# mutiann/few-shot-transformer-tts

Hardware: AMD Instinct MI355X
Metric: padded mel-frames/sec, full training step (fwd+loss+bwd+allreduce+Adam) (higher is better)
Workload: dtype bf16; 1 GPU; LJSpeech-shaped (BASELINE configs[1]) packed batch per GPU: B=14 S=114 T=582, default hparams (83.5M params), dropout on, single speaker/language; global_batch=14, seq_len=582, parallelism=dp1

## Files before the change

few-shot-transformer-tts_amd/b2s_hip/lib.py:

```python
import ctypes as C
import os

os.environ.setdefault("GPU_MAX_HW_QUEUES", "8")

import torch

_HERE = os.path.dirname(os.path.abspath(__file__))
LIB_PATH = os.environ.get("B2S_LIB_PATH") or os.path.join(os.path.dirname(_HERE), "libb2s_hip.so")

_lib = None


class B2SError(RuntimeError):
    pass


class Config(C.Structure):
    _fields_ = [(n, C.c_int32) for n in (
        "num_mels", "vocab_size", "embed_size", "encoder_hidden", "decoder_hidden",
        "n_encoder_layer", "n_decoder_layer", "n_attention_head",
        "prenet_hidden", "postnet_hidden", "n_postnet_layer",
        "multi_speaker", "max_num_speaker", "speaker_embedding_size",
        "multi_lingual", "max_num_language", "language_embedding_size")] + [
        ("transformer_dropout_rate", C.c_float), ("decoder_dropout_rate", C.c_float),
        ("reg_weight", C.c_float), ("compute_dtype", C.c_int32),
        ("guided_attention_weight", C.c_float), ("guided_attention_sigma", C.c_float), ("freeze_encoder", C.c_int32)]


class GemmDesc(C.Structure):
    _fields_ = [(n, C.c_int32) for n in ("dtype", "trans_a", "trans_b", "M", "N", "K", "lda", "ldb", "ldc", "c_fp32",
                                         "batch", "batch_inner")] + \
               [(n, C.c_int64) for n in ("a_bs_o", "a_bs_i", "b_bs_o", "b_bs_i", "c_bs_o", "c_bs_i")] + \
               [("alpha", C.c_float), ("relu", C.c_int32), ("accumulate", C.c_int32), ("drop_p", C.c_float),
                ("seed", C.c_uint64), ("conv_cin_a", C.c_int32), ("conv_T", C.c_int32), ("conv_dw_cin", C.c_int32),
                ("rows_per_batch", C.c_int32)]


P = C.c_void_p
_PROTOS = {
    "b2s_last_error": (C.c_char_p, []),
    "b2s_version": (C.c_int, []),
    "b2s_model_create": (C.c_int, [C.POINTER(Config), C.POINTER(P)]),
    "b2s_model_destroy": (None, [P]),
    "b2s_model_num_tensors": (C.c_int, [P]),
    "b2s_model_tensor_info": (C.c_int, [P, C.c_int, C.c_char_p, C.c_int, C.POINTER(C.c_int64), C.POINTER(C.c_int), C.POINTER(C.c_int)]),
    "b2s_model_bind": (C.c_int, [P, C.POINTER(P), C.POINTER(P), C.c_int]),
    "b2s_model_sync_weights": (C.c_int, [P, P, C.c_int]),
    "b2s_encoder_ws_bytes": (C.c_size_t, [P, C.c_int, C.c_int]),
    "b2s_encoder_forward": (C.c_int, [P, P, P, P, P, C.c_int, C.c_int, C.c_int, C.c_uint64, P, C.c_size_t, P, P, C.POINTER(P)]),
    "b2s_encoder_backward": (C.c_int, [P, P, P, P]),
    "b2s_decoder_ws_bytes": (C.c_size_t, [P, C.c_int, C.c_int, C.c_int]),
    "b2s_decoder_forward": (C.c_int, [P, P, P, P, P, C.c_int, C.c_int, C.c_int, C.c_int, C.c_uint64, P, C.c_size_t, P, P, P, P, C.POINTER(P)]),
    "b2s_decoder_backward": (C.c_int, [P, P, P, P, P, C.c_int, P, P, P]),
    "b2s_decoder_guided_loss": (C.c_int, [P, P, P, P, P]),
    "b2s_decoder_alignment": (C.c_int, [P, P, C.c_int, C.c_int, P, P]),
    "b2s_postnet_ws_bytes": (C.c_size_t, [P, C.c_int, C.c_int]),
    "b2s_postnet_forward": (C.c_int, [P, P, P, P, C.c_int, C.c_int, C.c_int, C.c_uint64, P, C.c_size_t, P, P, C.POINTER(P)]),
    "b2s_postnet_backward": (C.c_int, [P, P, P, P, C.c_int, P]),
    "b2s_ctx_free": (None, [P]),
    "b2s_loss_forward": (C.c_int, [P, P, P, P, P, P, C.c_int, C.c_int, P, P, P, P]),
    "b2s_loss_backward": (C.c_int, [P, P, P, P, P, P, C.c_int, C.c_int, P, P, P, P, P]),
    "b2s_l2_backward": (C.c_int, [P, P, P]),
    "b2s_adam_bind": (C.c_int, [P, C.POINTER(P), C.POINTER(P), C.c_int]),
    "b2s_adam_step": (C.c_int, [P, C.c_float, C.c_int, C.c_float, C.c_float, C.c_float, C.c_float, C.c_float, P]),
    "b2s_zero_grads": (C.c_int, [P, P, C.c_int]),
    "b2s_model_set_grad_slot_padding": (C.c_int, [P, C.c_int]),
    "b2s_gemm": (C.c_int, [C.POINTER(GemmDesc), P, P, P, P, P, P, P, P]),
    "b2s_gemm_splitk": (C.c_int, [C.POINTER(GemmDesc), C.c_int, P, P, P, P, C.c_size_t, P]),
    "b2s_layernorm_forward": (C.c_int, [C.c_int, P, P, P, P, P, P, C.c_int, C.c_int, C.c_float, P]),
    "b2s_layernorm_backward": (C.c_int, [C.c_int, P, P, P, P, P, P, P, P, C.c_int, C.c_int, P]),
    "b2s_attention_ws_bytes": (C.c_size_t, [C.c_int, C.c_int, C.c_int, C.c_int, C.c_int]),
    "b2s_attention_forward": (C.c_int, [C.c_int, P, C.c_int, P, C.c_int, P, C.c_int, P, C.c_int, C.c_int, C.c_int, C.c_int,
                                        C.c_int, C.c_int, C.c_int, P, P, C.c_int64, C.c_int64, C.c_float, C.c_uint64, P, P, P, P]),
    "b2s_attention_backward": (C.c_int, [C.c_int, P, C.c_int, P, C.c_int, P, C.c_int, P, C.c_int, P, P, P, C.c_int, P, C.c_int,
                                         P, C.c_int, C.c_int, C.c_int, C.c_int, C.c_int, C.c_int, C.c_float, C.c_uint64, P, P]),
    "b2s_flash_attention_forward": (C.c_int, [C.c_int, P, C.c_int, P, C.c_int, P, C.c_int, P, C.c_int, C.c_int, C.c_int, C.c_int, C.c_int,
                                              C.c_int, C.c_int, P, C.c_float, C.c_uint64, P, P]),
    "b2s_flash_attention_backward": (C.c_int, [C.c_int, P, P, C.c_int, P, C.c_int, P, C.c_int, P, C.c_int, P, P, P, C.c_int, P, C.c_int,
                                               P, C.c_int, C.c_int, C.c_int, C.c_int, C.c_int, C.c_int, C.c_int, P, C.c_float,
                                               C.c_uint64, P]),
    "b2s_flash_attention_align": (C.c_int, [C.c_int, P, C.c_int, P, C.c_int, P, C.c_int, C.c_int, C.c_int, C.c_int, C.c_int, C.c_int, P, P,
                                            P]),
    "b2s_align_from_probs": (C.c_int, [C.c_int, P, P, C.c_int, C.c_int, C.c_int, C.c_int, P]),
    "b2s_add3": (C.c_int, [P, P, P, P, C.c_int64, P]),
    "b2s_cast": (C.c_int, [C.c_int, P, P, C.c_int64, P]),
    "b2s_cast_back": (C.c_int, [C.c_int, P, P, C.c_int64, P]),
    "b2s_decode_ws_bytes": (C.c_size_t, [P, C.c_int, C.c_int, C.c_int, C.c_int]),
    "b2s_decode_begin": (C.c_int, [P, P, P, C.c_int, C.c_int, C.c_int, C.c_int, C.c_uint64, C.c_int, P, C.c_size_t, P, C.POINTER(P)]),
    "b2s_decode_run": (C.c_int, [P, P, C.c_int, C.c_int, P]),
    "b2s_decode_status": (C.c_int, [P, C.POINTER(C.c_int), C.POINTER(C.c_int), P]),
    "b2s_decode_fetch": (C.c_int, [P, P, C.c_int, P, P, P]),
    "b2s_decode_alignment": (C.c_int, [P, P, C.c_int, C.c_int, C.c_int, P, P]),
    "b2s_decode_end": (None, [P]),
    "b2s_model_second_stream": (C.c_void_p, [P]),
    "b2s_model_set_side_stream": (C.c_int, [P, P]),
    "b2s_gemm_set_tile_policy": (C.c_int, [C.c_int]),
    "b2s_model_backward_abort": (C.c_int, [P, P]),
    "b2s_model_mark_grads_ready": (C.c_int, [P]),
    "b2s_adam_shard": (C.c_int, [P, P, C.POINTER(C.c_int64), C.POINTER(C.c_int64), C.c_int]),
    "b2s_param_wire": (C.c_int, [P, P, C.c_int, P]),
    "b2s_model_set_stage_hook": (C.c_int, [P, P, P, P]),
    "b2s_prof_enable": (None, [C.c_int]),
    "b2s_adam_set_grad_wire": (C.c_int, [P, P, P]),
    "b2s_adam_step_groups": (C.c_int, [P, C.c_float, C.c_int, C.c_float, C.c_float, C.c_float, C.c_float, C.c_float, C.c_int, C.c_int, P]),
    "b2s_prof_collect": (C.c_int, [C.POINTER(C.c_double), C.c_int]),
    "b2s_dropout_mask": (C.c_int, [C.c_float, C.c_uint64, C.c_uint32, P, C.c_int64, P]),
    "b2s_decoder_compact_rows": (C.c_int, [P, P, C.c_int]),
    "b2s_dropout_mask_attn": (C.c_int, [C.c_float, C.c_uint64, C.c_uint32, P, C.c_int64, C.c_int, P]),
    "b2s_dropout_site": (C.c_int, [C.c_char_p, C.c_int, C.c_int, C.POINTER(C.c_uint32), C.POINTER(C.c_int), C.POINTER(C.c_int)]),
    "b2s_encf_attention_forward": (C.c_int, [P, P, P, P, C.c_int, C.c_int, C.c_float, C.c_uint64, C.c_uint32, P, P, P, P, C.c_int, P]),
    "b2s_encf_attention_backward": (C.c_int, [P, P, P, P, P, P, P, C.c_int, C.c_int, C.c_float, C.c_uint64, C.c_uint32, P, P, C.c_int, P]),
    "b2s_encf_ffn_sublayer": (C.c_int, [C.c_int, P, P, P, P, P, C.c_int, C.c_int, C.c_float, C.c_uint64, C.c_uint32, P, C.c_int, P]),
    "b2s_encf_reduce_layernorm_forward": (C.c_int, [P, P, C.c_int, C.c_int, C.c_float, C.c_uint64, C.c_uint32, P, P, P, P, P, C.c_int, P, P, C.c_int, P]),
    "b2s_encf_reduce_layernorm_backward": (C.c_int, [P, C.c_int, C.c_int, P, P, P, P, P, P, P, P, P, C.c_float, C.c_uint64, C.c_uint32, C.c_int, P]),
    "b2s_transpose_bf16": (C.c_int, [P, P, C.c_int, C.c_int, P]),
}
EXPORTS = sorted(_PROTOS)

# ... 35 lines not shown
```

few-shot-transformer-tts_amd/b2s_hip/ops.py:

```python
import ctypes as C

import torch

from . import lib as L


def _rup8(x):
    return (x + 7) // 8 * 8


def to_compute(x, dtype):
    x = x.contiguous()
    if not dtype:
        return x
    out = torch.empty(x.shape, dtype=torch.int16, device=x.device)
    L.check(L.load().b2s_cast(1, L.ptr(x), L.ptr(out), x.numel(), L.stream()))
    return out


def from_compute(x, dtype):
    if not dtype:
        return x
    out = torch.empty(x.shape, dtype=torch.float32, device=x.device)
    L.check(L.load().b2s_cast_back(1, L.ptr(x), L.ptr(out), x.numel(), L.stream()))
    return out


def gemm(dtype, A, B, M, N, K, trans_a=False, trans_b=False, out=None, c_fp32=True, lda=None, ldb=None, ldc=None,
         bias=None, relu=False, residual=None, accumulate=False, alpha=1.0, batch=1, batch_inner=1,
         a_bs=(0, 0), b_bs=(0, 0), c_bs=(0, 0), row_len=None, rows_per_batch=1, conv_cin_a=0, conv_T=0, conv_len=None,
         conv_dw_cin=0, drop_p=0.0, seed=0):
    d = L.GemmDesc()
    d.dtype, d.trans_a, d.trans_b, d.M, d.N, d.K = dtype, int(trans_a), int(trans_b), M, N, K
    d.lda = lda if lda is not None else (M if trans_a else K)
    d.ldb = ldb if ldb is not None else (N if trans_b else K)
    d.ldc = ldc if ldc is not None else N
    d.c_fp32 = int(c_fp32)
    d.batch, d.batch_inner = batch, batch_inner
    d.a_bs_o, d.a_bs_i = a_bs
    d.b_bs_o, d.b_bs_i = b_bs
    d.c_bs_o, d.c_bs_i = c_bs
    d.alpha, d.relu, d.accumulate, d.drop_p, d.seed = alpha, int(relu), int(accumulate), drop_p, seed
    d.conv_cin_a, d.conv_T, d.conv_dw_cin, d.rows_per_batch = conv_cin_a, conv_T, conv_dw_cin, rows_per_batch
    if out is None:
        shape = (batch, M, d.ldc) if batch > 1 else (M, d.ldc)
        out = torch.empty(shape, dtype=torch.float32 if c_fp32 or not dtype else torch.int16, device=A.device)
    L.check(L.load().b2s_gemm(C.byref(d), L.ptr(A), L.ptr(B), L.ptr(out), L.ptr(bias), L.ptr(residual), L.ptr(row_len),
                              L.ptr(conv_len), L.stream()))
    return out


class LinearFn(torch.autograd.Function):

    @staticmethod
    def forward(ctx, x, weight, bias, relu, dtype):
        K = x.shape[-1]
        N = weight.shape[0]
        x2 = x.reshape(-1, K)
        M = x2.shape[0]
        xT, wT = to_compute(x2, dtype), to_compute(weight, dtype)
        y = gemm(dtype, xT, wT, M, N, K, bias=bias.contiguous() if bias is not None else None, relu=relu)
        ctx.save_for_backward(xT, wT, y if relu else None)
        ctx.dtype, ctx.shape, ctx.has_bias, ctx.relu = dtype, x.shape, bias is not None, relu
        return y.reshape(x.shape[:-1] + (N,))

    @staticmethod
    def backward(ctx, dy):
        xT, wT, y = ctx.saved_tensors
        dtype = ctx.dtype
        M, K = xT.shape
        N = wT.shape[0]
        dy2 = dy.reshape(M, N)
        if ctx.relu:
            dy2 = dy2 * (y > 0)
        dyT = to_compute(dy2, dtype)
        dx = gemm(dtype, dyT, wT, M, K, N, trans_b=True)
        dw = gemm(dtype, dyT, xT, N, K, M, trans_a=True, trans_b=True)
        db = None
        if ctx.has_bias:
            ones = to_compute(torch.ones(M, 8, device=dy.device), dtype)
            db = gemm(dtype, dyT, ones, N, 8, M, trans_a=True, trans_b=True)[:, 0].contiguous()
        return dx.reshape(ctx.shape), dw, db, None, None


def linear(x, weight, bias=None, relu=False, dtype=0):
    return LinearFn.apply(x, weight, bias, relu, dtype)


class LayerNormFn(torch.autograd.Function):
    @staticmethod
    def forward(ctx, x, weight, bias, eps, dtype):
        D = x.shape[-1]
        x2 = x.reshape(-1, D).contiguous()
        M = x2.shape[0]
        y = torch.empty(M, D, dtype=torch.int16 if dtype else torch.float32, device=x.device)
        mean = torch.empty(M, dtype=torch.float32, device=x.device)
        rstd = torch.empty_like(mean)
        L.check(L.load().b2s_layernorm_forward(dtype, L.ptr(x2), L.ptr(weight), L.ptr(bias), L.ptr(y), L.ptr(mean),
                                               L.ptr(rstd), M, D, eps, L.stream()))
        ctx.save_for_backward(x2, weight, mean, rstd)
        ctx.dtype, ctx.shape = dtype, x.shape
        return from_compute(y, dtype).reshape(x.shape)

    @staticmethod
    def backward(ctx, dy):
        x2, weight, mean, rstd = ctx.saved_tensors
        M, D = x2.shape
        dyT = to_compute(dy.reshape(M, D), ctx.dtype)
        dx = torch.empty_like(x2)
        dg = torch.empty(D, dtype=torch.float32, device=x2.device)
        db = torch.empty_like(dg)
        L.check(L.load().b2s_layernorm_backward(ctx.dtype, L.ptr(dyT), L.ptr(x2), L.ptr(weight), L.ptr(mean), L.ptr(rstd),
                                                L.ptr(dx), L.ptr(dg), L.ptr(db), M, D, L.stream()))
        return dx.reshape(ctx.shape), dg, db, None, None


def dropout_mask(shape, p, seed, op_id, device):
    n = 1
    for d in shape:
        n *= int(d)
    m = torch.empty(n, dtype=torch.uint8, device=device)
    L.check(L.load().b2s_dropout_mask(float(p), int(seed), int(op_id), L.ptr(m), n, L.stream()))
    return m.reshape(shape).to(torch.float32) * (1.0 / (1.0 - p))


def layernorm(x, weight, bias, eps=1e-6, dtype=0):
# ... 96 lines not shown
```

few-shot-transformer-tts_amd/csrc/b2s_common.h:

```cpp
#pragma once
#include <hip/hip_runtime.h>
#include <stdint.h>
#include <stdio.h>
#include <string.h>

typedef uint16_t bf16_t;

typedef __attribute__((ext_vector_type(8))) short bf16x8_t;
typedef __attribute__((ext_vector_type(4))) short bf16x4_t;
typedef __attribute__((ext_vector_type(4))) float f32x4_t;

#define B2S_WAVE 64

extern thread_local char g_b2s_err[512];
int b2s_fail(const char* file, int line, const char* fmt, ...);
#define B2S_CHECK(cond, ...) do { if (!(cond)) return b2s_fail(__FILE__, __LINE__, __VA_ARGS__); } while (0)
#define B2S_HIP(expr) do { hipError_t e_ = (expr); if (e_ != hipSuccess) \
    return b2s_fail(__FILE__, __LINE__, "HIP error %d (%s) in %s", (int)e_, hipGetErrorString(e_), #expr); } while (0)
#define B2S_LAUNCH_CHECK() B2S_HIP(hipGetLastError())
#define B2S_TRY(expr) do { int r_ = (expr); if (r_) return r_; } while (0)

__device__ __host__ inline float bf2f(bf16_t x) {
    union { uint32_t u; float f; } c; c.u = ((uint32_t)x) << 16; return c.f;
}
__device__ inline uint32_t f2bf2(float lo, float hi) {
    typedef __bf16 bf2_t __attribute__((ext_vector_type(2)));
    typedef float f2_t __attribute__((ext_vector_type(2)));
    const f2_t v = {lo, hi};
    const bf2_t w = __builtin_convertvector(v, bf2_t);
    return __builtin_bit_cast(uint32_t, w);
}
__device__ __host__ inline bf16_t f2bf(float f) {
#if defined(__HIP_DEVICE_COMPILE__)
    return (bf16_t)(f2bf2(f, 0.f) & 0xffffu);
#endif
    union { uint32_t u; float f; } c; c.f = f;
    uint32_t u = c.u;
    if ((u & 0x7fffffffu) > 0x7f800000u) return (bf16_t)0x7fc0;
    u += 0x7fffu + ((u >> 16) & 1u);
    return (bf16_t)(u >> 16);
}

template <typename T> struct TT;
template <> struct TT<float> {
    static constexpr int VE = 4;
    __device__ static inline float ld(const float* p) { return *p; }
    __device__ static inline void st(float* p, float v) { *p = v; }
};
template <> struct TT<bf16_t> {
    static constexpr int VE = 8;
    __device__ static inline float ld(const bf16_t* p) { return bf2f(*p); }
    __device__ static inline void st(bf16_t* p, float v) { *p = f2bf(v); }
};

__device__ __host__ inline uint32_t b2s_hash32(uint32_t x) {
    x ^= x >> 16; x *= 0x7feb352dU; x ^= x >> 15; x *= 0x846ca68bU; x ^= x >> 16; return x;
}
struct DropCfg {
    uint32_t key;
    uint32_t thresh;
    float scale;
};
__device__ __host__ inline bool b2s_keep(const DropCfg& d, uint32_t idx) {
    return b2s_hash32(idx * 0x9E3779B1u + d.key) >= d.thresh;
}
constexpr uint32_t B2S_WC0 = 0x85EBCA6Bu, B2S_WC1 = 0xC2B2AE35u;
__device__ __host__ inline uint32_t b2s_wseed(const DropCfg& d, uint32_t row) { return b2s_hash32(row * 0x9E3779B1u + d.key); }
__device__ __host__ inline uint32_t b2s_wmix(uint32_t seed, uint32_t kq) { const uint32_t x = seed + kq * 0x9E3779B1u; return x ^ (x >> 16); }
__device__ __host__ inline int b2s_wthresh(const DropCfg& d) { return (int)(d.thresh >> 16) - 32768; }
__device__ __host__ inline bool b2s_keep_w(const DropCfg& d, uint32_t row, uint32_t k) {
    const uint32_t w = b2s_wmix(b2s_wseed(d, row), k >> 2) * ((k & 2u) ? B2S_WC1 : B2S_WC0);
    return (int)(int16_t)(uint16_t)(w >> ((k & 1u) * 16u)) >= b2s_wthresh(d);
}
inline DropCfg make_drop(float p, uint64_t seed, uint32_t op_id) {
    DropCfg d;
    if (p <= 0.f) { d.key = 0; d.thresh = 0; d.scale = 1.f; return d; }
    d.key = b2s_hash32((uint32_t)seed ^ b2s_hash32((uint32_t)(seed >> 32) + 0x51ed270bU) ^ (op_id * 0x85ebca6bU + 0x1234567U));
    double t = (double)p * 4294967296.0;
    d.thresh = t >= 4294967295.0 ? 0xffffffffu : (uint32_t)t;
    d.scale = 1.f / (1.f - p);
    return d;
}

__device__ inline float wave_sum(float v) {
#pragma unroll
    for (int o = 32; o > 0; o >>= 1) v += __shfl_xor(v, o, 64);
    return v;
}
__device__ inline float wave_max(float v) {
#pragma unroll
    for (int o = 32; o > 0; o >>= 1) v = fmaxf(v, __shfl_xor(v, o, 64));
    return v;
}

static inline int cdiv(long a, long b) { return (int)((a + b - 1) / b); }
```

few-shot-transformer-tts_amd/csrc/capi_ops.hip:

```cpp
#include "engine.h"
#include "attention.h"
#include "enc_fused.h"

namespace {
inline hipStream_t S_(void* s) { return (hipStream_t)s; }
inline int rup8(int x) { return (x + 7) & ~7; }
__global__ void k_dropmask(DropCfg d, uint8_t* out, long n) {
    long i = (long)blockIdx.x * blockDim.x + threadIdx.x;
    if (i < n) out[i] = b2s_keep(d, (uint32_t)i) ? 1 : 0;
}
}

int b2s_attn_core_fwd_export(int dtype, hipStream_t st, const void* q, int ldq, const void* k, int ldk, const void* v, int ldv,
                             void* ctx, int ldc, int B, int H, int Lq, int Lk, int dh, int mask_mode, const int* klen,
                             const float* bias, long bias_sb, long bias_sq, DropCfg drop, float* S, void* P, void* Pd);
int b2s_attn_core_bwd_export(int dtype, hipStream_t st, const void* dctx, int ldc, const void* q, int ldq, const void* k, int ldk,
                             const void* v, int ldv, const void* P, const void* Pd, void* dq, int lddq, void* dk, int lddk,
                             void* dv, int lddv, int B, int H, int Lq, int Lk, int dh, DropCfg drop, float* dP, void* dS);

extern "C" int b2s_gemm(const b2s_gemm_desc* d, const void* A, const void* B, void* C, const float* bias,
                        const float* residual, const int32_t* row_len, const int32_t* conv_len, void* stream) {
    B2S_CHECK(d && A && B && C, "null argument");
    GemmArgs g;
    g.M = d->M; g.N = d->N; g.K = d->K; g.batch = d->batch > 0 ? d->batch : 1; g.batch_inner = d->batch_inner > 0 ? d->batch_inner : 1;
    g.A.p = A; g.A.ld = d->lda; g.A.bs_o = d->a_bs_o; g.A.bs_i = d->a_bs_i;
    g.B.p = B; g.B.ld = d->ldb; g.B.bs_o = d->b_bs_o; g.B.bs_i = d->b_bs_i;
    if (d->trans_a) { g.A.R = d->K; g.A.C = d->M; } else { g.A.R = d->M; g.A.C = d->K; }
    if (d->trans_b) { g.B.R = d->K; g.B.C = d->N; } else { g.B.R = d->N; g.B.C = d->K; }
    if (d->conv_cin_a > 0) {
        B2S_CHECK(!d->trans_a, "conv gather is defined on the row-major A operand");
        g.A.g_cin = d->conv_cin_a; g.A.g_T = d->conv_T; g.A.g_len = conv_len; g.A.R = d->M; g.A.C = d->K;
    }
    g.C = C; g.c_fp32 = d->c_fp32; g.ldc = d->ldc; g.cs_o = d->c_bs_o; g.cs_i = d->c_bs_i;
    g.epi.alpha = d->alpha; g.epi.bias = bias; g.epi.relu = d->relu; g.epi.accumulate = d->accumulate;
    g.epi.drop = make_drop(d->drop_p, d->seed, 7u);
    g.epi.residual = residual; g.epi.ldr = d->ldc;
    g.epi.row_len = row_len; g.epi.rows_per_batch = d->rows_per_batch > 0 ? d->rows_per_batch : 1;
    g.epi.conv_dw_cin = d->conv_dw_cin;
    if (d->conv_dw_cin > 0 && d->conv_T > 0 && d->conv_cin_a == 0) {
        B2S_CHECK(d->dtype == 1 && d->trans_a && d->trans_b && g.batch == 1 && d->c_fp32 && d->alpha == 1.f && !bias && !residual && !row_len && !d->relu &&
                  d->drop_p == 0.f, "conv dW on token rows: bf16 TN form, fp32 output, linear epilogue");
        B2S_CHECK(d->N == 5 * d->conv_dw_cin && d->K % d->conv_T == 0, "conv dW on token rows: N = %d must be 5 cin (cin = %d), K = %d a multiple of T = %d",
                  d->N, d->conv_dw_cin, d->K, d->conv_T);
        GemmArgs w;
        w.A.p = A; w.A.ld = d->lda; w.B.p = B; w.B.ld = d->ldb; w.M = d->M; w.N = d->conv_dw_cin; w.K = d->K;
        w.C = C; w.c_fp32 = 1; w.ldc = d->ldc; w.epi.accumulate = d->accumulate;
        return b2s_gemm_conv_dw_launch(&w, 1, conv_len, d->K / d->conv_T, d->conv_T, S_(stream));
    }
    return b2s_gemm_launch(g, d->dtype, d->trans_a != 0, d->trans_b != 0, S_(stream));
}
extern "C" int b2s_gemm_splitk(const b2s_gemm_desc* d, int splitk, const void* A, const void* B, float* C, float* ws, size_t ws_floats,
                               void* stream) {
    B2S_CHECK(d && A && B && C && splitk >= 1, "null argument / bad split");
    B2S_CHECK(d->c_fp32 && d->accumulate && !d->relu && d->drop_p == 0.f && d->conv_cin_a == 0, "split-K needs a linear fp32 accumulate epilogue");
    GemmArgs g;
    g.M = d->M; g.N = d->N; g.K = d->K; g.batch = d->batch > 0 ? d->batch : 1; g.batch_inner = d->batch_inner > 0 ? d->batch_inner : 1;
    g.A.p = A; g.A.ld = d->lda; g.A.bs_o = d->a_bs_o; g.A.bs_i = d->a_bs_i;
    g.B.p = B; g.B.ld = d->ldb; g.B.bs_o = d->b_bs_o; g.B.bs_i = d->b_bs_i;
    if (d->trans_a) { g.A.R = d->K; g.A.C = d->M; } else { g.A.R = d->M; g.A.C = d->K; }
    if (d->trans_b) { g.B.R = d->K; g.B.C = d->N; } else { g.B.R = d->N; g.B.C = d->K; }
    g.C = C; g.c_fp32 = 1; g.ldc = d->ldc; g.cs_o = d->c_bs_o; g.cs_i = d->c_bs_i;
    g.epi.alpha = d->alpha; g.epi.accumulate = 1; g.epi.conv_dw_cin = d->conv_dw_cin;
    g.splitk = splitk; g.ws = ws; g.ws_floats = ws ? ws_floats : 0;
    return b2s_gemm_launch(g, d->dtype, d->trans_a != 0, d->trans_b != 0, S_(stream));
}
extern "C" int b2s_layernorm_forward(int dtype, const float* x, const float* gamma, const float* beta, void* y, float* mean,
                                     float* rstd, int M, int D, float eps, void* stream) {
    B2S_CHECK(x && gamma && beta && y && mean && rstd, "null argument");
    return ro_layernorm_fwd(dtype, x, gamma, beta, y, D, nullptr, 0, mean, rstd, M, D, eps, nullptr, 1, S_(stream));
}
extern "C" int b2s_layernorm_backward(int dtype, const void* dy, const float* x, const float* gamma, const float* mean,
                                      const float* rstd, float* dx, float* dgamma, float* dbeta, int M, int D, void* stream) {
    B2S_CHECK(dy && x && gamma && mean && rstd && dx && dgamma && dbeta, "null argument");
    B2S_HIP(hipMemsetAsync(dgamma, 0, sizeof(float) * D, S_(stream)));
    B2S_HIP(hipMemsetAsync(dbeta, 0, sizeof(float) * D, S_(stream)));
    return ro_layernorm_bwd(dtype, dy, 0, D, x, gamma, mean, rstd, dx, 0, dgamma, dbeta, M, D, nullptr, 1, S_(stream));
}
extern "C" size_t b2s_attention_ws_bytes(int dtype, int B, int H, int Lq, int Lk) {
    const size_t pn = (size_t)B * H * Lq * rup8(Lk);
    return 2 * pn * 4 + pn * (dtype ? 2 : 4) + 1024;
}
extern "C" int b2s_attention_forward(int dtype, const void* q, int ldq, const void* k, int ldk, const void* v, int ldv, void* ctx,
                                     int ldc, int B, int H, int Lq, int Lk, int dh, int mask_mode, const int32_t* klen,
                                     const float* bias, int64_t bias_sb, int64_t bias_sq, float drop_p, uint64_t seed, void* ws,
                                     void* P_out, void* Pd_out, void* stream) {
    B2S_CHECK(q && k && v && ctx && ws && P_out, "null argument");
    B2S_CHECK(drop_p <= 0.f || Pd_out, "Pd_out is required when dropout is on");
    return b2s_attn_core_fwd_export(dtype, S_(stream), q, ldq, k, ldk, v, ldv, ctx, ldc, B, H, Lq, Lk, dh, mask_mode, klen, bias,
                                    bias_sb, bias_sq, make_drop(drop_p, seed, 11u), (float*)ws, P_out, Pd_out);
}
extern "C" int b2s_attention_backward(int dtype, const void* dctx, int ldc, const void* q, int ldq, const void* k, int ldk,
                                      const void* v, int ldv, const void* P, const void* Pd, void* dq, int lddq, void* dk, int lddk,
                                      void* dv, int lddv, int B, int H, int Lq, int Lk, int dh, float drop_p, uint64_t seed, void* ws,
                                      void* stream) {
    B2S_CHECK(dctx && q && k && v && P && dq && dk && dv && ws, "null argument");
    const size_t pn = (size_t)B * H * Lq * rup8(Lk);
    float* dP = (float*)ws + pn;
    void* dS = (void*)((float*)ws + 2 * pn);
    return b2s_attn_core_bwd_export(dtype, S_(stream), dctx, ldc, q, ldq, k, ldk, v, ldv, P, Pd, dq, lddq, dk, lddk, dv, lddv, B, H,
                                    Lq, Lk, dh, make_drop(drop_p, seed, 11u), dP, dS);
}
namespace {
AttnArgs mk_args(const void* q, int ldq, const void* k, int ldk, const void* v, int ldv, int B, int H, int Lq, int Lk, int dh, int mask_mode,
                 const int32_t* klen, float drop_p, uint64_t seed, float* lse) {
    AttnArgs a;
    a.q = q; a.k = k; a.v = v; a.ldq = ldq; a.ldk = ldk; a.ldv = ldv; a.B = B; a.H = H; a.Lq = Lq; a.Lk = Lk;
    a.scale = 1.f / sqrtf((float)dh); a.mask_mode = mask_mode; a.klen = klen; a.drop = make_drop(drop_p, seed, 11u); a.lse = lse;
    return a;
}
}
extern "C" int b2s_flash_attention_forward(int dtype, const void* q, int ldq, const void* k, int ldk, const void* v, int ldv, void* ctx, int ldc,
                                           int B, int H, int Lq, int Lk, int dh, int mask_mode, const int32_t* klen, float drop_p,
                                           uint64_t seed, float* lse_out, void* stream) {
    B2S_CHECK(ctx && lse_out, "null argument");
    AttnArgs a = mk_args(q, ldq, k, ldk, v, ldv, B, H, Lq, Lk, dh, mask_mode, klen, drop_p, seed, lse_out);
    a.out = ctx; a.ldo = ldc;
    return b2s_flash_fwd(dtype, a, dh, S_(stream));
}
extern "C" int b2s_flash_attention_backward(int dtype, const void* dctx, const void* ctx, int ldc, const void* q, int ldq, const void* k, int ldk,
                                            const void* v, int ldv, const float* lse, float* dsum_scratch, void* dq, int lddq, void* dk,
                                            int lddk, void* dv, int lddv, int B, int H, int Lq, int Lk, int dh, int mask_mode,
                                            const int32_t* klen, float drop_p, uint64_t seed, void* stream) {
    B2S_CHECK(dctx && ctx && lse && dsum_scratch, "null argument");
    AttnArgs a = mk_args(q, ldq, k, ldk, v, ldv, B, H, Lq, Lk, dh, mask_mode, klen, drop_p, seed, const_cast<float*>(lse));
    a.dout = dctx; a.ldo = ldc; a.dsum = dsum_scratch; a.dq = dq; a.dk = dk; a.dv = dv; a.lddq = lddq; a.lddk = lddk; a.lddv = lddv;
    return b2s_flash_bwd(dtype, a, dh, ctx, S_(stream));
}
extern "C" int b2s_flash_attention_align(int dtype, const void* q, int ldq, const void* k, int ldk, const float* lse, int B, int H, int Lq, int Lk,
                                         int dh, int mask_mode, const int32_t* klen, float* align_out, void* stream) {
    AttnArgs a = mk_args(q, ldq, k, ldk, nullptr, 0, B, H, Lq, Lk, dh, mask_mode, klen, 0.f, 0, const_cast<float*>(lse));
    return b2s_flash_align(dtype, a, dh, align_out, S_(stream));
// ... 83 lines not shown
```

few-shot-transformer-tts_amd/csrc/engine.hip:

```cpp
#include <algorithm>
#include <cmath>
#include <cstdarg>
#include <cstdlib>
#include "engine.h"
#include "attention.h"
#include "enc_fused.h"
#include "drop_sites.h"

thread_local char g_b2s_err[512] = "";
int b2s_fail(const char* file, int line, const char* fmt, ...) {
    char msg[400];
    va_list ap; va_start(ap, fmt); vsnprintf(msg, sizeof(msg), fmt, ap); va_end(ap);
    const char* base = strrchr(file, '/');
    snprintf(g_b2s_err, sizeof(g_b2s_err), "%s:%d: %s", base ? base + 1 : file, line, msg);
    return 1;
}

int b2s_model::id(const std::string& n) const {
    auto it = index.find(n);
    return it == index.end() ? -1 : it->second;
}

namespace {

// ... 1738 lines not shown
    return ro_align_transpose(m->dtype, s.P, out, c->B * m->cfg.n_attention_head, s.Lq, s.Lk, s.ldp, S_(stream));
}

extern "C" size_t b2s_postnet_ws_bytes(const b2s_model* m, int B, int T) {
    if (!m || B <= 0 || T <= 0) return 0;
    b2s_ctx c; c.B = B; c.T = T;
    Arena a; PostScratch ps;
    plan_postnet(m, c, a, ps);
    return a.off + 4096;
}

extern "C" int b2s_postnet_forward(b2s_model* m, const float* inputs, const int32_t* lengths, const float* add, int B, int T,
                                   int train, uint64_t seed, void* ws, size_t ws_bytes, float* out, void* stream,
                                   b2s_ctx** ctx_out) {
    B2S_TRY(check_bound(m));
    const b2s_config& cf = m->cfg;
    B2S_CHECK(inputs && lengths && out && ws && B > 0 && T > 0, "bad argument");
    hipStream_t st = S_(stream);
    b2s_ctx* c = new b2s_ctx();
    c->kind = 3; c->B = B; c->T = T; c->train = train; c->seed = seed; c->tgt_len = lengths;
    c->ws = (char*)ws; c->ws_bytes = ws_bytes;
    Arena a; a.base = (char*)ws; a.cap = ws_bytes;
    PostScratch ps;
    plan_postnet(m, *c, a, ps);
    if (a.overflow || a.off > ws_bytes) { delete c; return b2s_fail(__FILE__, __LINE__, "postnet workspace too small: need %zu bytes, got %zu", a.off, ws_bytes); }
    const long M = (long)B * T;
    const int n = cf.n_postnet_layer, dt = m->dtype;
    const float pd = train ? cf.decoder_dropout_rate : 0.f;
    const bool fused_stats = train && M > 1;
    auto run = [&]() -> int {
        B2S_TRY(ro_cast(dt, inputs, c->u[0], M * cf.num_mels, st));
        if (fused_stats) B2S_HIP(hipMemsetAsync(ps.stat, 0, sizeof(float) * (size_t)n * ps.stat_stride, st));
        for (int i = 0; i < n; ++i) {
            const int cin = i == 0 ? cf.num_mels : cf.postnet_hidden, cout = i == n - 1 ? cf.num_mels : cf.postnet_hidden;
            const std::string q = "postnet.batchnorm_layers." + std::to_string(i) + ".";
            float* sums = ps.stat + (size_t)i * ps.stat_stride;
            GemmArgs g;
            g.A.p = c->u[i]; g.A.ld = cin; g.A.R = (int)M; g.A.C = 5 * cin; g.A.g_cin = cin; g.A.g_T = T; g.A.g_len = lengths;
            g.B.p = m->conv_wf[i]; g.B.ld = 5 * cin; g.B.R = cout; g.B.C = 5 * cin;
            g.M = (int)M; g.N = cout; g.K = 5 * cin; g.C = c->y[i]; g.c_fp32 = 1; g.ldc = cout;
            if (fused_stats) g.epi.colstat = sums;
            B2S_TRY(b2s_gemm_launch(g, dt, false, false, st));
            DropCfg d = make_drop(pd, seed, drop_op(DS_POST_CONV, i));
            const bool last = i == n - 1;
            if (fused_stats) {
                B2S_TRY(ro_bn_apply_train(dt, c->y[i], sums, c->bn_mean[i], c->bn_rstd[i], 1e-5f, m->P(q + "running_mean"), m->P(q + "running_var"),
                                          (long*)m->data[m->id(q + "num_batches_tracked")], 0.1f, m->P(q + "weight"), m->P(q + "bias"), last ? 0 : 1,
                                          last ? nullptr : c->u[i + 1], last ? out : nullptr, last ? add : nullptr, (int)M, cout, d, st));
                continue;
            }
            if (train)
                B2S_TRY(ro_bn_stats(c->y[i], (int)M, cout, c->bn_mean[i], c->bn_rstd[i], 1e-5f, m->P(q + "running_mean"),
                                    m->P(q + "running_var"), (long*)m->data[m->id(q + "num_batches_tracked")], 0.1f, sums, st));
            else
                B2S_TRY(ro_bn_eval_stats(m->P(q + "running_mean"), m->P(q + "running_var"), c->bn_mean[i], c->bn_rstd[i], 1e-5f, cout, st));
            if (!last)
                B2S_TRY(ro_bn_apply(dt, c->y[i], c->bn_mean[i], c->bn_rstd[i], m->P(q + "weight"), m->P(q + "bias"), 1, c->u[i + 1],
                                    nullptr, nullptr, (int)M, cout, d, st));
            else
                B2S_TRY(ro_bn_apply(dt, c->y[i], c->bn_mean[i], c->bn_rstd[i], m->P(q + "weight"), m->P(q + "bias"), 0, nullptr, out,
                                    add, (int)M, cout, d, st));
        }
        return 0;
    };
    int rc = run();
    if (rc || !ctx_out) { delete c; if (ctx_out) *ctx_out = nullptr; return rc; }
    *ctx_out = c;
    return 0;
}

extern "C" int b2s_postnet_backward(b2s_model* m, b2s_ctx* c, const float* d_out, float* d_inputs_out, int flags, void* stream) {
    B2S_TRY(check_bound(m));
    B2S_CHECK(c && c->kind == 3 && d_out && d_inputs_out, "bad postnet context");
    B2S_CHECK(c->train, "postnet backward requires a train-mode forward (batch statistics)");
    const b2s_config& cf = m->cfg;
    hipStream_t st = S_(stream);
    const int B = c->B, T = c->T, n = cf.n_postnet_layer, dt = m->dtype;
    const long M = (long)B * T;
    const float pd = cf.decoder_dropout_rate;
    Arena a; a.base = c->ws; a.cap = c->ws_bytes;
    b2s_ctx tmp; tmp.B = B; tmp.T = T;
    PostScratch ps;
    plan_postnet(m, tmp, a, ps);
    std::vector<GemmArgs> dws, segs;
    for (int i = n - 1; i >= 0; --i) {
        const int cin = i == 0 ? cf.num_mels : cf.postnet_hidden, cout = i == n - 1 ? cf.num_mels : cf.postnet_hidden;
        const std::string q = "postnet.batchnorm_layers." + std::to_string(i) + ".";
        DropCfg d = make_drop(pd, c->seed, drop_op(DS_POST_CONV, i));
        const void* dout = i == n - 1 ? (const void*)d_out : ps.du[i + 1];
        void* dy = ps.dy[i];
        B2S_TRY(ro_bn_bwd(dt, dout, i == n - 1 ? 1 : 0, c->y[i], c->bn_mean[i], c->bn_rstd[i], m->P(q + "weight"), m->P(q + "bias"),
                          i < n - 1 ? 1 : 0, m->G(q + "weight"), m->G(q + "bias"), dy, (int)M, cout, d, st));
        if (dt == 1 && cin % 8 == 0 && cout % 8 == 0) {
            GemmArgs g;
            g.A.p = dy; g.A.ld = cout; g.B.p = c->u[i]; g.B.ld = cin;
            g.M = cout; g.N = cin; g.K = (int)M;
            g.C = m->G("postnet.conv_layers." + std::to_string(i) + ".weight"); g.c_fp32 = 1; g.ldc = 5 * cin;
            g.epi.accumulate = 1;
            segs.push_back(g);
        } else {
            GemmArgs g;
            g.A.p = dy; g.A.ld = cout; g.A.R = (int)M; g.A.C = cout;
            g.B.p = c->u[i]; g.B.ld = cin; g.B.R = (int)M; g.B.C = 5 * cin; g.B.g_cin = cin; g.B.g_T = T; g.B.g_len = c->tgt_len;
            g.M = cout; g.N = 5 * cin; g.K = (int)M;
            g.C = m->G("postnet.conv_layers." + std::to_string(i) + ".weight"); g.c_fp32 = 1; g.ldc = 5 * cin;
            g.epi.conv_dw_cin = cin; g.epi.accumulate = 1; g.splitk = pick_splitk(cout, 5 * cin, (int)M, dt);
            if (m->aux) dws.push_back(g);
            else { m->set_ws(g, st); B2S_TRY(b2s_gemm_launch(g, dt, true, true, st)); }
        }
        {
            GemmArgs g;
            g.A.p = dy; g.A.ld = cout; g.A.R = (int)M; g.A.C = 5 * cout; g.A.g_cin = cout; g.A.g_T = T; g.A.g_len = nullptr;
            g.B.p = m->conv_wb[i]; g.B.ld = 5 * cout; g.B.R = cin; g.B.C = 5 * cout;
            g.M = (int)M; g.N = cin; g.K = 5 * cout;
            g.epi.row_len = c->tgt_len; g.epi.rows_per_batch = T;
            if (i == 0) { g.C = d_inputs_out; g.c_fp32 = 1; } else { g.C = ps.du[i]; g.c_fp32 = 0; }
            g.ldc = cin;
            B2S_TRY(b2s_gemm_launch(g, dt, false, false, st));
        }
    }
    auto launch_segs = [&](hipStream_t s) -> int {
        for (size_t i = 0; i < segs.size(); i += B2S_MAX_GROUP)
            B2S_TRY(b2s_gemm_conv_dw_launch(segs.data() + i, (int)std::min<size_t>(B2S_MAX_GROUP, segs.size() - i), c->tgt_len, B, T, s));
        return 0;
    };
    if (!m->aux) B2S_TRY(launch_segs(st));
    else if (!dws.empty() || !segs.empty()) {
        hipEvent_t ready = m->next_event();
        B2S_HIP(hipEventRecord(ready, st));
        B2S_HIP(hipStreamWaitEvent(m->aux, ready, 0));
        for (GemmArgs& g : dws) { m->set_ws(g, m->aux); B2S_TRY(b2s_gemm_launch(g, dt, true, true, m->aux)); }
        B2S_TRY(launch_segs(m->aux));
        hipEvent_t done = m->next_event();
        B2S_HIP(hipEventRecord(done, m->aux));
        m->aux_dirty = true;
        m->pending_ev = done;
    }
    if ((flags & B2S_POST_BWD_DEFER_JOIN) && m->aux) {
        B2S_TRY(flush_ln_jobs(m, st));
        m->pending_stages.push_back(0);
        return 0;
    }
    B2S_TRY(join_aux(m, st));
    B2S_TRY(hook_after_stream(m, st));
    fire_stages(m, m->pending_stages);
    m->stage_done(0);
    m->pending_ev = nullptr;
    return 0;
}

extern "C" int b2s_loss_forward(b2s_model* m, const float* mel_bef, const float* mel_aft, const float* stop_logits,
                                const float* mel_targets, const int32_t* target_lengths, int B, int T, float* losses_out,
                                float* aft_losses_out, float* scratch, void* stream) {
    B2S_TRY(check_bound(m));
    B2S_CHECK(mel_bef && mel_aft && stop_logits && mel_targets && target_lengths && losses_out && aft_losses_out && scratch, "null argument");
    hipStream_t st = S_(stream);
    float* l2 = scratch;
    const bool fused_zero = m->l2_fresh;
    if (m->l2_fresh) {
        B2S_TRY(ro_sum_scaled(m->l2_part, m->n_adam_chunks, 0.5f * m->cfg.reg_weight, l2, st, scratch + 1, 3 + B));
    } else {
        B2S_HIP(hipMemsetAsync(l2, 0, sizeof(float), st));
        if (m->n_l2_chunks) B2S_TRY(ro_mt_sumsq(m->l2_chunks, m->n_l2_chunks, l2, 0.5f * m->cfg.reg_weight, st));
    }
    return ro_loss_fwd(mel_bef, mel_aft, stop_logits, mel_targets, target_lengths, l2, losses_out, aft_losses_out, B, T,
                       m->cfg.num_mels, 5.0f, scratch + 1, st, fused_zero);
}
extern "C" int b2s_loss_backward(b2s_model* m, const float* mel_bef, const float* mel_aft, const float* stop_logits,
                                 const float* mel_targets, const int32_t* target_lengths, int B, int T, const float* grad_scale,
                                 float* d_bef, float* d_aft, float* d_stop, void* stream) {
    B2S_CHECK(m && mel_bef && mel_aft && stop_logits && mel_targets && target_lengths && d_bef && d_aft && d_stop, "null argument");
    return ro_loss_bwd(mel_bef, mel_aft, stop_logits, mel_targets, target_lengths, grad_scale, d_bef, d_aft, d_stop, B, T,
                       m->cfg.num_mels, 5.0f, S_(stream));
}
extern "C" int b2s_l2_backward(b2s_model* m, const float* grad_scale, void* stream) {
    B2S_TRY(check_bound(m));
    for (size_t i = 0; i < m->tinfo.size(); ++i)
        B2S_CHECK(!m->tinfo[i].l2 || m->grad[i], "gradient of %s is not bound", m->tinfo[i].name.c_str());
    return ro_mt_axpy(m->l2_chunks, m->n_l2_chunks, m->cfg.reg_weight, grad_scale, S_(stream));
}
extern "C" int b2s_adam_bind(b2s_model* m, void* const* exp_avg_host, void* const* exp_avg_sq_host, int n) {
    B2S_TRY(check_bound(m));
    B2S_CHECK(n == (int)m->tinfo.size() && exp_avg_host && exp_avg_sq_host, "expected %d state pointers", (int)m->tinfo.size());
    for (int i = 0; i < n; ++i) {
        m->exp_avg[i] = exp_avg_host[i]; m->exp_avg_sq[i] = exp_avg_sq_host[i];
        B2S_CHECK(m->tinfo[i].kind != 1 || !m->grad[i] || (m->exp_avg[i] && m->exp_avg_sq[i]), "missing Adam state for %s", m->tinfo[i].name.c_str());
    }
    return rebuild_adam_chunks(m);
}
extern "C" int b2s_adam_set_grad_wire(b2s_model* m, const void* wire_bf16, const float* grad_base) {
    B2S_CHECK(m && (!wire_bf16 || grad_base), "null argument");
    B2S_CHECK(!wire_bf16 || (((size_t)wire_bf16 & 15) == 0 && ((size_t)grad_base & 15) == 0), "wire / gradient buffers must be 16-byte aligned");
    m->adam_wire = wire_bf16; m->adam_gbase = wire_bf16 ? grad_base : nullptr;
    return 0;
}
namespace {
AdamHyper adam_hyper(float lr, int step, float beta1, float beta2) {
    return AdamHyper{lr, (float)(1.0 - std::pow((double)beta1, step)), (float)std::sqrt(1.0 - std::pow((double)beta2, step))};
}
}
// ... 153 lines not shown
```

few-shot-transformer-tts_amd/csrc/gemm.h:

```cpp
#pragma once
#include "b2s_common.h"

struct GemmOperand {
    const void* p = nullptr;
    long bs_o = 0, bs_i = 0;
    int ld = 0;
    int R = 0, C = 0;
    int g_cin = 0, g_T = 0;
    const int* g_len = nullptr;
};

struct GemmEpilogue {
    float alpha = 1.f;
    const float* bias = nullptr;
    int relu = 0;
    const void* relu_aux = nullptr;
    int ld_aux = 0;
    float aux_scale = 1.f;
    DropCfg drop = {0, 0, 1.f};
    const int* drop_salt = nullptr;
    const float* residual = nullptr;
    int ldr = 0;
    const int* row_len = nullptr;
    int rows_per_batch = 1;
    int conv_dw_cin = 0;
    int accumulate = 0;
    float* colstat = nullptr;
    void *kv_k = nullptr, *kv_v = nullptr;
    const int* kv_t = nullptr;
    int kv_maxT = 0, kv_D = 0, kv_dh = 0;
};

struct GemmArgs {
    GemmOperand A, B;
    int M = 0, N = 0, K = 0;
    int batch = 1, batch_inner = 1;
    int splitk = 1;
    void* C = nullptr;
    int c_fp32 = 0;
    int ldc = 0;
    long cs_o = 0, cs_i = 0;
    GemmEpilogue epi;
    float* ws = nullptr;
    size_t ws_floats = 0;
};

int b2s_gemm_launch(const GemmArgs& g, int dtype, bool ta, bool tb, hipStream_t stream);
int b2s_gemm_glds_launch(const GemmArgs& g, bool ta, bool tb, hipStream_t stream);
int b2s_gemm_skinny_launch(const GemmArgs& g, int dtype, hipStream_t stream);
long b2s_gemm_glds256_tiles(const GemmArgs& g);
int b2s_gemm_glds256_launch(const GemmArgs& g, bool ta, bool tb, const bf16_t* zero, hipStream_t stream);
int b2s_splitk_reduce_launch(const float* ws, float* dst, int M, int N, int ldc, int splitk, int conv_dw_cin, hipStream_t stream);
#define B2S_MAX_GROUP 8
struct b2s_gemm_group { int n; int order; int tile0[B2S_MAX_GROUP + 1]; GemmArgs p[B2S_MAX_GROUP];
                        const int* seg_len; int seg_n, seg_T; };
int b2s_gemm_glds256_grouped_launch(const GemmArgs* probs, int n, const bf16_t* zero, hipStream_t stream);
int b2s_gemm_glds256_conv_dw_launch(const GemmArgs* probs, int n, const int* len, int B, int T, const bf16_t* zero, hipStream_t stream);
int b2s_gemm_conv_dw_launch(const GemmArgs* probs, int n, const int* len, int B, int T, hipStream_t stream);
const bf16_t* b2s_gemm_zero_page();
int b2s_gemm_grouped_launch(const GemmArgs* probs, int n, hipStream_t stream);
```

few-shot-transformer-tts_amd/csrc/gemm.hip:

```cpp
#include <mutex>
#include "gemm.h"
#include "gemm_epi.h"

namespace {

constexpr int BM = 128, BN = 128;

constexpr int BK = 16, KSTEP = 4, VE = 4;

__device__ inline float frag_n(const float* tile, int LD, int row0, int k0, int i, int g) {
    return tile[(row0 + i) * LD + k0 + g];
}
__device__ inline float frag_t(const float* tile, int LD, int row0, int k0, int i, int g) {
    return tile[(k0 + g) * LD + row0 + i];
}
__device__ inline f32x4_t mma(float a, float b, f32x4_t c) {
    return __builtin_amdgcn_mfma_f32_16x16x4f32(a, b, c, 0, 0, 0);
}

template <typename T>
__device__ inline uint4 load_chunk(const GemmOperand& o, const T* base, int r, int c) {
    uint4 z = make_uint4(0, 0, 0, 0);
    if (o.g_cin > 0) {
        if (r >= o.R || c >= o.C) return z;
// ... 183 lines not shown
}

#include <atomic>
#include <vector>
#include <cstdlib>
namespace {
struct ProfRec { hipEvent_t a, b; int variant; double flops; int M, N, K, batch, splitk; };
std::atomic<bool> g_prof_on{false};
std::mutex g_prof_mu;
std::vector<ProfRec> g_prof;
}
extern "C" void b2s_prof_enable(int on) { g_prof_on = on != 0; }
extern "C" int b2s_prof_collect(double* out, int n_variants) {
    for (int i = 0; i < n_variants * 3; ++i) out[i] = 0.0;
    std::lock_guard<std::mutex> lock(g_prof_mu);
    for (auto& r : g_prof) {
        B2S_HIP(hipEventSynchronize(r.b));
        float ms = 0.f;
        B2S_HIP(hipEventElapsedTime(&ms, r.a, r.b));
        if (r.variant < n_variants) { out[r.variant * 3] += r.flops; out[r.variant * 3 + 1] += ms; out[r.variant * 3 + 2] += 1.0; }
        (void)hipEventDestroy(r.a); (void)hipEventDestroy(r.b);
    }
    g_prof.clear();
    return 0;
}

static int gemm_launch_inner(const GemmArgs& g, int dtype, bool ta, bool tb, hipStream_t stream);
int b2s_gemm_launch(const GemmArgs& g, int dtype, bool ta, bool tb, hipStream_t stream) {
    if (!g_prof_on) return gemm_launch_inner(g, dtype, ta, tb, stream);
    ProfRec r;
    B2S_HIP(hipEventCreate(&r.a)); B2S_HIP(hipEventCreate(&r.b));
    r.variant = dtype * 8 + (ta ? 4 : 0) + (tb ? 2 : 0) + ((g.A.g_cin > 0 || g.B.g_cin > 0) ? 1 : 0);
    r.flops = 2.0 * g.M * g.N * (double)g.K * g.batch;
    r.M = g.M; r.N = g.N; r.K = g.K; r.batch = g.batch; r.splitk = g.splitk;
    B2S_HIP(hipEventRecord(r.a, stream));
    int rc = gemm_launch_inner(g, dtype, ta, tb, stream);
    B2S_HIP(hipEventRecord(r.b, stream));
    { std::lock_guard<std::mutex> lock(g_prof_mu); g_prof.push_back(r); }
    return rc;
}
int b2s_gemm_grouped_launch(const GemmArgs* probs, int n, hipStream_t stream) {
    if (!g_prof_on) return b2s_gemm_glds256_grouped_launch(probs, n, b2s_gemm_zero_page(), stream);
    ProfRec r;
    B2S_HIP(hipEventCreate(&r.a)); B2S_HIP(hipEventCreate(&r.b));
    r.variant = 16; r.flops = 0.0;
    for (int i = 0; i < n; ++i) r.flops += 2.0 * probs[i].M * probs[i].N * (double)probs[i].K;
    r.M = probs[0].M; r.N = probs[0].N; r.K = probs[0].K; r.batch = n; r.splitk = 1;
    B2S_HIP(hipEventRecord(r.a, stream));
    int rc = b2s_gemm_glds256_grouped_launch(probs, n, b2s_gemm_zero_page(), stream);
    B2S_HIP(hipEventRecord(r.b, stream));
    { std::lock_guard<std::mutex> lock(g_prof_mu); g_prof.push_back(r); }
    return rc;
}
int b2s_gemm_conv_dw_launch(const GemmArgs* probs, int n, const int* len, int B, int T, hipStream_t stream) {
    const bf16_t* zero = b2s_gemm_zero_page();
    if (!zero) return 1;
    if (!g_prof_on) return b2s_gemm_glds256_conv_dw_launch(probs, n, len, B, T, zero, stream);
    ProfRec r;
    B2S_HIP(hipEventCreate(&r.a)); B2S_HIP(hipEventCreate(&r.b));
    r.variant = 16; r.flops = 0.0;
    for (int i = 0; i < n; ++i) r.flops += 2.0 * probs[i].M * 5.0 * probs[i].N * (double)B * T;
    r.M = probs[0].M; r.N = 5 * probs[0].N; r.K = B * T; r.batch = n; r.splitk = 1;
    B2S_HIP(hipEventRecord(r.a, stream));
    int rc = b2s_gemm_glds256_conv_dw_launch(probs, n, len, B, T, zero, stream);
    B2S_HIP(hipEventRecord(r.b, stream));
    { std::lock_guard<std::mutex> lock(g_prof_mu); g_prof.push_back(r); }
    return rc;
}
static int gemm_launch_inner(const GemmArgs& g, int dtype, bool ta, bool tb, hipStream_t stream) {
    const int ve = dtype ? 8 : 4;
    B2S_CHECK(g.M > 0 && g.N > 0 && g.K > 0 && g.batch > 0 && g.batch_inner > 0, "gemm: bad shape M=%d N=%d K=%d batch=%d",
              g.M, g.N, g.K, g.batch);
    B2S_CHECK(g.A.p && g.B.p && g.C, "gemm: null pointer");
    B2S_CHECK(g.A.ld % ve == 0 && g.B.ld % ve == 0, "gemm: leading dimensions (%d, %d) must be multiples of %d", g.A.ld,
              g.B.ld, ve);
    B2S_CHECK(((uintptr_t)g.A.p % 16 == 0) && ((uintptr_t)g.B.p % 16 == 0), "gemm: operands must be 16-byte aligned");
    B2S_CHECK(g.A.bs_o % ve == 0 && g.A.bs_i % ve == 0 && g.B.bs_o % ve == 0 && g.B.bs_i % ve == 0,
              "gemm: batch strides must be multiples of %d elements", ve);
    B2S_CHECK(g.batch * g.splitk <= 65535, "gemm: batch too large");
    B2S_CHECK(g.splitk >= 1 && (g.splitk == 1 || (g.c_fp32 && g.epi.accumulate && !g.epi.relu && !g.epi.bias && !g.epi.residual &&
                                                   !g.epi.relu_aux && !g.epi.drop.thresh)),
              "gemm: split-K needs a linear fp32 accumulate epilogue");
    B2S_CHECK(!g.epi.kv_k, "gemm: the cache-append fusion exists in the decode-step kernel only (M <= 64, K %% 32 == 0)");
    if (!dtype) return launch_fp32(g, ta, tb, stream);
    static const long min_m = getenv("B2S_GEMM256_MIN_M") ? atol(getenv("B2S_GEMM256_MIN_M")) : 129;
    if (g.batch == 1 && g.M >= min_m) {
        const bf16_t* zero = b2s_gemm_zero_page();
        if (!zero) return 1;
        return b2s_gemm_glds256_launch(g, ta, tb, zero, stream);
    }
    return b2s_gemm_glds_launch(g, ta, tb, stream);
}
```

few-shot-transformer-tts_amd/csrc/gemm_epi.h:

```cpp
#pragma once
#include "gemm.h"

__device__ __forceinline__ void epi_store16(void* p, uint4 v) { *reinterpret_cast<uint4*>(p) = v; }
template <int NBv>
__device__ __forceinline__ void epi_colstat(const f32x4_t (&acc)[4][NBv], float* colstat, float alpha, int M, int N, int mb, int nb, int lane) {
    const int li = lane & 15, lg = lane >> 4;
#pragma unroll
    for (int b = 0; b < NBv; ++b) {
        float s1 = 0.f, s2 = 0.f;
#pragma unroll
        for (int a = 0; a < 4; ++a)
#pragma unroll
            for (int r = 0; r < 4; ++r) {
                const float v = (mb + a * 16 + lg * 4 + r) < M ? acc[a][b][r] * alpha : 0.f;
                s1 += v; s2 += v * v;
            }
        s1 += __shfl_xor(s1, 16, 64); s1 += __shfl_xor(s1, 32, 64);
        s2 += __shfl_xor(s2, 16, 64); s2 += __shfl_xor(s2, 32, 64);
        const int n = nb + b * 16 + li;
        if (lg == 0 && n < N) { atomicAdd(colstat + n, s1); atomicAdd(colstat + N + n, s2); }
    }
}

#ifndef B2S_EPI_FAST
// ... 5 lines not shown
    const float* residual; int ldr;
    const void* relu_aux; int ld_aux; float aux_scale;
    DropCfg drop; const int* drop_salt;
};
template <int NB, int MODE>
__device__ __forceinline__ void gemm_wave_epilogue_fast(const EpiFast g, f32x4_t (&acc)[4][NB], float* stg, int mb, int nb, int lane, int z, long cbase) {
    constexpr int CH = NB * 2;
    const int li = lane & 15, lg = lane >> 4;
    const EpiFast& e = g;
    int trow[CH], tcol[CH];
#pragma unroll
    for (int k = 0; k < CH; ++k) { const int id = k * 64 + lane; trow[k] = id / CH; tcol[k] = (id - trow[k] * CH) * 8; }
    typedef uint32_t epi_u32x4 __attribute__((ext_vector_type(4)));
    f32x4_t r0[MODE == 3 ? CH : 1], r1[MODE == 3 ? CH : 1];
    epi_u32x4 qa[MODE == 2 ? CH : 1];
    constexpr bool EARLY = NB <= 3;
    auto load_res = [&]() {
#pragma unroll
        for (int k = 0; k < CH; ++k) {
            const float* rp = e.residual + (long)(mb + trow[k]) * e.ldr + nb + tcol[k];
            r0[k] = *reinterpret_cast<const f32x4_t*>(rp); r1[k] = *reinterpret_cast<const f32x4_t*>(rp + 4);
        }
    };
    if (MODE == 3 && EARLY) load_res();
    if (MODE == 2) {
        const bf16_t* aux = reinterpret_cast<const bf16_t*>(e.relu_aux);
#pragma unroll
        for (int k = 0; k < CH; ++k) qa[k] = *reinterpret_cast<const epi_u32x4*>(aux + (long)(mb + trow[k]) * e.ld_aux + nb + tcol[k]);
    }
    __builtin_amdgcn_s_barrier();
#pragma unroll
    for (int a = 0; a < 4; ++a)
#pragma unroll
        for (int r = 0; r < 4; ++r) {
            const int row = a * 16 + lg * 4 + r;
#pragma unroll
            for (int b = 0; b < NB; ++b) stg[row * 64 + ((b * 16 + li) ^ (((row >> 2) & 1) << 4))] = acc[a][b][r];
        }
    __builtin_amdgcn_sched_barrier(0);
    if (MODE == 3 && !EARLY) load_res();
    DropCfg dcfg = e.drop;
    if (e.drop.thresh && e.drop_salt) dcfg.key ^= b2s_hash32((uint32_t)(*e.drop_salt) * 2246822519u + 3266489917u);
    float* Cf = reinterpret_cast<float*>(g.C);
    bf16_t* Ct = reinterpret_cast<bf16_t*>(g.C);
#pragma unroll
    for (int k = 0; k < CH; ++k) {
        const int row = trow[k], m = mb + row, n = nb + tcol[k];
        const f32x4_t v0 = *reinterpret_cast<const f32x4_t*>(stg + row * 64 + (tcol[k] ^ (((row >> 2) & 1) << 4)));
        const f32x4_t v1 = *reinterpret_cast<const f32x4_t*>(stg + row * 64 + (tcol[k] ^ (((row >> 2) & 1) << 4)) + 4);
        float v[8] = {v0[0], v0[1], v0[2], v0[3], v1[0], v1[1], v1[2], v1[3]};
        if (MODE == 1) {
#pragma unroll
            for (int j = 0; j < 8; ++j) v[j] = fmaxf(v[j], 0.f);
        }
        if (MODE == 2) {
            const uint32_t w[4] = {qa[k][0], qa[k][1], qa[k][2], qa[k][3]};
#pragma unroll
            for (int j = 0; j < 8; ++j) {
                const uint32_t bits = (w[j >> 1] >> ((j & 1) * 16)) & 0xffffu;
                v[j] = (bits != 0 && !(bits & 0x8000u)) ? v[j] * e.aux_scale : 0.f;
            }
        }
        if ((MODE == 1 || MODE == 3) && dcfg.thresh) {
            const uint32_t idx = (uint32_t)(((long)z * g.M + m) * g.N + n);
#pragma unroll
            for (int j = 0; j < 8; ++j) v[j] = b2s_keep(dcfg, idx + j) ? v[j] * dcfg.scale : 0.f;
        }
        const long off = cbase + (long)m * g.ldc + n;
        if (MODE == 4) {
            const f32x4_t o0 = {v[0], v[1], v[2], v[3]}, o1 = {v[4], v[5], v[6], v[7]};
            *reinterpret_cast<f32x4_t*>(Cf + off) = o0; *reinterpret_cast<f32x4_t*>(Cf + off + 4) = o1;
        } else if (MODE == 3) {
            const f32x4_t o0 = {v[0] + r0[k][0], v[1] + r0[k][1], v[2] + r0[k][2], v[3] + r0[k][3]};
            const f32x4_t o1 = {v[4] + r1[k][0], v[5] + r1[k][1], v[6] + r1[k][2], v[7] + r1[k][3]};
            *reinterpret_cast<f32x4_t*>(Cf + off) = o0; *reinterpret_cast<f32x4_t*>(Cf + off + 4) = o1;
        } else {
            const epi_u32x4 o = {f2bf2(v[0], v[1]), f2bf2(v[2], v[3]), f2bf2(v[4], v[5]), f2bf2(v[6], v[7])};
            *reinterpret_cast<epi_u32x4*>(Ct + off) = o;
        }
    }
}

template <int NB>
__device__ __forceinline__ void gemm_wave_epilogue(GemmArgs g, f32x4_t (&acc)[4][NB], float* stg, int mb, int nb, int lane, int z, int zo, int zi,
                                          int ksplit, float* splitk_ws) {
    const int li = lane & 15, lg = lane >> 4;
    if (g.epi.colstat && g.splitk == 1) epi_colstat<NB>(acc, g.epi.colstat, g.epi.alpha, g.M, g.N, mb, nb, lane);
#if B2S_EPI_FAST
    {
        const GemmEpilogue& e = g.epi;
        const long cb = zo * g.cs_o + zi * g.cs_i;
        const bool common = g.splitk == 1 && e.conv_dw_cin == 0 && !e.accumulate && !e.bias && !e.row_len && e.alpha == 1.f && !e.kv_k &&
                            mb + 64 <= g.M && nb + NB * 16 <= g.N && (g.ldc & 7) == 0 && (cb & 7) == 0 &&
                            (reinterpret_cast<uintptr_t>(g.C) & 15) == 0;
        if (common) {
            const EpiFast f = {g.C, g.ldc, g.M, g.N, e.residual, e.ldr, e.relu_aux, e.ld_aux, e.aux_scale, e.drop, e.drop_salt};
            if (!g.c_fp32 && !e.residual) {
                if (!e.relu && !e.relu_aux && !e.drop.thresh) { gemm_wave_epilogue_fast<NB, 0>(f, acc, stg, mb, nb, lane, z, cb); return; }
                if (e.relu && !e.relu_aux) { gemm_wave_epilogue_fast<NB, 1>(f, acc, stg, mb, nb, lane, z, cb); return; }
                if (e.relu_aux && !e.relu && !e.drop.thresh && (e.ld_aux & 7) == 0 && (reinterpret_cast<uintptr_t>(e.relu_aux) & 15) == 0) {
                    gemm_wave_epilogue_fast<NB, 2>(f, acc, stg, mb, nb, lane, z, cb); return;
                }
            } else if (g.c_fp32 && e.residual && !e.relu && !e.relu_aux && (e.ldr & 3) == 0 && (reinterpret_cast<uintptr_t>(e.residual) & 15) == 0) {
                gemm_wave_epilogue_fast<NB, 3>(f, acc, stg, mb, nb, lane, z, cb); return;
            } else if (g.c_fp32 && !e.residual && !e.relu && !e.relu_aux && !e.drop.thresh) {
                gemm_wave_epilogue_fast<NB, 4>(f, acc, stg, mb, nb, lane, z, cb); return;
            }
        }
    }
#endif
    GemmEpilogue e = g.epi;
    if (g.splitk > 1 && splitk_ws) {
        g.C = splitk_ws + (long)ksplit * g.M * g.N; g.c_fp32 = 1; g.ldc = g.N; g.cs_o = 0; g.cs_i = 0; g.splitk = 1;
        e.accumulate = 0; e.conv_dw_cin = 0;
    }
    if (g.splitk > 1 || e.conv_dw_cin > 0) {
        float* Cw = reinterpret_cast<float*>(g.C) + zo * g.cs_o + zi * g.cs_i;
#pragma unroll
        for (int a = 0; a < 4; ++a)
#pragma unroll
            for (int r = 0; r < 4; ++r) {
                const int m = mb + a * 16 + lg * 4 + r;
                if (m >= g.M) continue;
#pragma unroll
                for (int b = 0; b < NB; ++b) {
                    int nn = nb + b * 16 + li;
                    if (nn >= g.N) continue;
                    if (e.conv_dw_cin > 0) { int jj = nn / e.conv_dw_cin; nn = (nn - jj * e.conv_dw_cin) * 5 + jj; }
                    const float v = acc[a][b][r] * e.alpha;
                    float* dst = Cw + (long)m * g.ldc + nn;
                    if (g.splitk > 1) atomicAdd(dst, v); else if (e.accumulate) *dst += v; else *dst = v;
                }
            }
        return;
    }
    __builtin_amdgcn_s_barrier();
#pragma unroll
    for (int a = 0; a < 4; ++a)
#pragma unroll
        for (int r = 0; r < 4; ++r) {
            const int row = a * 16 + lg * 4 + r;
#pragma unroll
            for (int b = 0; b < NB; ++b) stg[row * 64 + ((b * 16 + li) ^ (((row >> 2) & 1) << 4))] = acc[a][b][r];
        }
    __builtin_amdgcn_sched_barrier(0);
    const long cbase = zo * g.cs_o + zi * g.cs_i;
    float* Cf = reinterpret_cast<float*>(g.C);
    bf16_t* Ct = reinterpret_cast<bf16_t*>(g.C);
    const bf16_t* aux = reinterpret_cast<const bf16_t*>(e.relu_aux);
    DropCfg dcfg = e.drop;
    if (e.drop.thresh && e.drop_salt) dcfg.key ^= b2s_hash32((uint32_t)(*e.drop_salt) * 2246822519u + 3266489917u);
    const bool vec_ok = (g.ldc & 7) == 0 && (cbase & 7) == 0 && e.conv_dw_cin == 0 && g.splitk == 1 &&
                        ((reinterpret_cast<uintptr_t>(g.C) & 15) == 0);
    const int cchunk = lane & 7;
    const int n = nb + cchunk * 8;
    float bv[8];
#pragma unroll
    for (int j = 0; j < 8; ++j) bv[j] = (e.bias && n + j < g.N) ? e.bias[n + j] : 0.f;
    const bool full = n + 8 <= g.N;
    const bool lane_ok = n < g.N && cchunk < NB * 2;
    const bool pre_res = e.residual && full && (e.ldr & 3) == 0;
    const bool pre_acc = !e.residual && vec_ok && full && g.c_fp32 && e.accumulate;
    const bool pre_aux = aux && full && (e.ld_aux & 7) == 0;
    constexpr int PG = 4;
#pragma unroll
    for (int pg = 0; pg < 8; pg += PG) {
    float4 q0[PG], q1[PG];
    uint4 qa[PG];
#pragma unroll
    for (int pp = 0; pp < PG; ++pp) {
        const int m = mb + (pg + pp) * 8 + (lane >> 3);
        q0[pp] = q1[pp] = make_float4(0.f, 0.f, 0.f, 0.f);
        qa[pp] = make_uint4(0, 0, 0, 0);
        if (m >= g.M || !lane_ok) continue;
        if (pre_res) {
// ... 5 lines not shown
        }
        if (pre_aux) qa[pp] = *reinterpret_cast<const uint4*>(aux + (long)m * e.ld_aux + n);
    }
#pragma unroll
    for (int pp = 0; pp < PG; ++pp) {
        const int p = pg + pp;
        const int row = p * 8 + (lane >> 3);
        const int m = mb + row;
        const float4 v0 = *reinterpret_cast<const float4*>(stg + row * 64 + ((cchunk * 8) ^ (((row >> 2) & 1) << 4)));
        const float4 v1 = *reinterpret_cast<const float4*>(stg + row * 64 + ((cchunk * 8) ^ (((row >> 2) & 1) << 4)) + 4);
        if (m >= g.M || n >= g.N || cchunk >= NB * 2) continue;
        float v[8] = {v0.x, v0.y, v0.z, v0.w, v1.x, v1.y, v1.z, v1.w};
#pragma unroll
        for (int j = 0; j < 8; ++j) v[j] = v[j] * e.alpha + bv[j];
        if (e.relu) {
#pragma unroll
            for (int j = 0; j < 8; ++j) v[j] = fmaxf(v[j], 0.f);
        }
        if (aux) {
            if (pre_aux) {
                const uint4 u = qa[pp];
                const uint32_t w[4] = {u.x, u.y, u.z, u.w};
#pragma unroll
                for (int j = 0; j < 8; ++j) {
                    const uint32_t bits = (w[j >> 1] >> ((j & 1) * 16)) & 0xffffu;
                    v[j] = (bits != 0 && !(bits & 0x8000u)) ? v[j] * e.aux_scale : 0.f;
                }
            } else {
#pragma unroll
                for (int j = 0; j < 8; ++j)
                    if (n + j < g.N) v[j] = bf2f(aux[(long)m * e.ld_aux + n + j]) > 0.f ? v[j] * e.aux_scale : 0.f;
            }
        }
        if (e.drop.thresh) {
            const uint32_t idx = (uint32_t)(((long)z * g.M + m) * g.N + n);
#pragma unroll
            for (int j = 0; j < 8; ++j) v[j] = b2s_keep(dcfg, idx + j) ? v[j] * dcfg.scale : 0.f;
        }
        if (e.residual) {
            if (pre_res) {
                const float4 r0 = q0[pp], r1 = q1[pp];
                v[0] += r0.x; v[1] += r0.y; v[2] += r0.z; v[3] += r0.w; v[4] += r1.x; v[5] += r1.y; v[6] += r1.z; v[7] += r1.w;
            } else {
#pragma unroll
                for (int j = 0; j < 8; ++j) if (n + j < g.N) v[j] += e.residual[(long)m * e.ldr + n + j];
            }
        }
        if (e.row_len) {
            const int bb = m / e.rows_per_batch, t = m - bb * e.rows_per_batch;
            if (t >= e.row_len[bb]) {
#pragma unroll
                for (int j = 0; j < 8; ++j) v[j] = 0.f;
            }
        }
        const long off = cbase + (long)m * g.ldc + n;
        if (vec_ok && full) {
            if (g.c_fp32) {
                float4* dst = reinterpret_cast<float4*>(Cf + off);
                float4 o0 = make_float4(v[0], v[1], v[2], v[3]), o1 = make_float4(v[4], v[5], v[6], v[7]);
                if (e.accumulate) {
                    const float4 c0 = pre_acc ? q0[pp] : dst[0], c1 = pre_acc ? q1[pp] : dst[1];
                    o0.x += c0.x; o0.y += c0.y; o0.z += c0.z; o0.w += c0.w; o1.x += c1.x; o1.y += c1.y; o1.z += c1.z; o1.w += c1.w;
                }
                epi_store16(dst, make_uint4(__float_as_uint(o0.x), __float_as_uint(o0.y), __float_as_uint(o0.z), __float_as_uint(o0.w)));
                epi_store16(dst + 1, make_uint4(__float_as_uint(o1.x), __float_as_uint(o1.y), __float_as_uint(o1.z), __float_as_uint(o1.w)));
            } else {
                uint4 o;
                o.x = f2bf2(v[0], v[1]); o.y = f2bf2(v[2], v[3]); o.z = f2bf2(v[4], v[5]); o.w = f2bf2(v[6], v[7]);
                epi_store16(Ct + off, o);
            }
        } else {
#pragma unroll
            for (int j = 0; j < 8; ++j) {
                if (n + j >= g.N) continue;
                int nn = n + j;
                if (e.conv_dw_cin > 0) { int jj = nn / e.conv_dw_cin; nn = (nn - jj * e.conv_dw_cin) * 5 + jj; }
                const long o = cbase + (long)m * g.ldc + nn;
                if (g.c_fp32) { if (g.splitk > 1) atomicAdd(Cf + o, v[j]); else if (e.accumulate) Cf[o] += v[j]; else Cf[o] = v[j]; }
                else Ct[o] = f2bf(v[j]);
            }
        }
    }
    }
}
```

few-shot-transformer-tts_amd/csrc/gemm_glds.hip:

```cpp
#include <algorithm>
#include <mutex>
#include "gemm.h"
#include "gemm_epi.h"

namespace {

constexpr int BM = 128, BN = 128, BK = 32;
constexpr int TILE = 128 * 32;
constexpr int NSTAGE = 4;

typedef __attribute__((address_space(1))) void* gptr_t;
typedef __attribute__((address_space(3))) void* lptr_t;
typedef __attribute__((address_space(3))) bf16x4_t* lds_b64_ptr;

__device__ inline int swz_t(int k) { return ((k & 3) | ((k >> 1) & 4)) << 1; }
__device__ inline int swz_n(int r) { return (-(r >> 2)) & 3; }

__device__ inline const bf16_t* chunk_src(const GemmOperand& o, const bf16_t* base, int r, int c, const bf16_t* zero) {
    if (r >= o.R || c >= o.C) return zero;
    if (o.g_cin > 0) {
        int j = c / o.g_cin, ci = c - j * o.g_cin;
        int b = r / o.g_T, t = r - b * o.g_T;
        int ts = t + j - 2;
        int lim = o.g_len ? min(o.g_len[b], o.g_T) : o.g_T;
// ... 52 lines not shown
                else    { int r = q * 16 + (lane >> 2), pc = lane & 3; int c = pc ^ swz_n(r);   sa = chunk_src(g.A, Ab, m0 + r, kb + c * 8, zero); }
                if (TB) { int kr = q * 4 + (lane >> 4), pc = lane & 15; int c = pc ^ swz_t(kr); sb = chunk_src(g.B, Bb, kb + kr, n0 + c * 8, zero); }
                else    { int r = q * 16 + (lane >> 2), pc = lane & 3; int c = pc ^ swz_n(r);   sb = chunk_src(g.B, Bb, n0 + r, kb + c * 8, zero); }
            } else {
                sa = (ka[i] >= 0 && kb + ka[i] < limA) ? pa[i] + kt * stepA : zero;
                sb = (kb_[i] >= 0 && kb + kb_[i] < limB) ? pb[i] + kt * stepB : zero;
            }
            __builtin_amdgcn_global_load_lds((gptr_t)sa, (lptr_t)(smem + buf * 2 * TILE + q * 512), 16, 0, 0);
            __builtin_amdgcn_global_load_lds((gptr_t)sb, (lptr_t)(smem + buf * 2 * TILE + TILE + q * 512), 16, 0, 0);
        }
    };
    unsigned offA[4], offB[4];
#pragma unroll
    for (int t = 0; t < 4; ++t) {
        if (TA) { const int k = lg * 8 + (li >> 2), col = wrow + t * 16 + (li & 3) * 4, sw = ((li >> 2) | ((lg & 1) << 2)) << 1;
                  offA[t] = 2u * (k * 128 + (((col >> 3) ^ sw) << 3) + (col & 7)); }
        else    { const int r = wrow + t * 16 + li; offA[t] = 2u * (r * 32 + ((lg ^ swz_n(r)) << 3)); }
        if (TB) { const int k = lg * 8 + (li >> 2), col = wcol + t * 16 + (li & 3) * 4, sw = ((li >> 2) | ((lg & 1) << 2)) << 1;
                  offB[t] = 2u * (TILE + k * 128 + (((col >> 3) ^ sw) << 3) + (col & 7)); }
        else    { const int r = wcol + t * 16 + li; offB[t] = 2u * (TILE + r * 32 + ((lg ^ swz_n(r)) << 3)); }
    }
    const unsigned lds_base = (unsigned)(uintptr_t)(lptr_t)smem;
    auto frag_issue = [&](bf16x8_t& dst, bool trans, unsigned addr) {
        if (!trans) {
            asm volatile("ds_read_b128 %0, %1" : "=v"(dst) : "v"(addr) : "memory");
        } else {
            bf16x4_t lo, hi;
            asm volatile("ds_read_b64_tr_b16 %0, %2\n\tds_read_b64_tr_b16 %1, %2 offset:1024"
                         : "=&v"(lo), "=&v"(hi) : "v"(addr) : "memory");
            dst[0] = lo[0]; dst[1] = lo[1]; dst[2] = lo[2]; dst[3] = lo[3];
            dst[4] = hi[0]; dst[5] = hi[1]; dst[6] = hi[2]; dst[7] = hi[3];
        }
    };

    f32x4_t acc[4][4];
#pragma unroll
    for (int a = 0; a < 4; ++a)
#pragma unroll
        for (int b = 0; b < 4; ++b) acc[a][b] = (f32x4_t){0.f, 0.f, 0.f, 0.f};

#define B2S_MMA16(CA, CB)                                                                                         \
    _Pragma("unroll") for (int a = 0; a < 4; ++a) _Pragma("unroll") for (int b = 0; b < 4; ++b)                   \
        acc[a][b] = __builtin_amdgcn_mfma_f32_16x16x32_bf16(CA[a], CB[b], acc[a][b], 0, 0, 0);
#define B2S_STEP(KT, CA, CB, NA, NB)                                                                              \
    {                                                                                                              \
        asm volatile("s_waitcnt vmcnt(%0)" ::"n"(4 * (NSTAGE - 3)) : "memory");       \
        __builtin_amdgcn_s_barrier();                          \
        issue(kt0 + (KT) + NSTAGE - 1, ((KT) + NSTAGE - 1) % NSTAGE);                                              \
        const unsigned sb_ = lds_base + (unsigned)((((KT) + 1) % NSTAGE) * 2 * TILE * 2);                         \
        _Pragma("unroll") for (int t = 0; t < 4; ++t) {                                                            \
            frag_issue(NA[t], TA, sb_ + offA[t]);                                                                  \
            frag_issue(NB[t], TB, sb_ + offB[t]);                                                                  \
        }                                                                                                          \
        __builtin_amdgcn_sched_barrier(0);                                                                         \
        B2S_MMA16(CA, CB)                                                                                          \
        __builtin_amdgcn_sched_barrier(0);              \
        asm volatile("s_waitcnt lgkmcnt(0)" ::: "memory");                 \
        __builtin_amdgcn_sched_barrier(0);                                                                         \
    }
#pragma unroll
    for (int p = 0; p < NSTAGE - 1; ++p) issue(kt0 + p, p);
    bf16x8_t fa0[4], fb0[4], fa1[4], fb1[4];
    asm volatile("s_waitcnt vmcnt(%0)" ::"n"(4 * (NSTAGE - 2)) : "memory");
    __builtin_amdgcn_s_barrier();
#pragma unroll
    for (int t = 0; t < 4; ++t) { frag_issue(fa0[t], TA, lds_base + offA[t]); frag_issue(fb0[t], TB, lds_base + offB[t]); }
    asm volatile("s_waitcnt lgkmcnt(0)" ::: "memory");
    __builtin_amdgcn_sched_barrier(0);
    int kt = 0;
    for (; kt + 2 < nk; kt += 2) {
        B2S_STEP(kt, fa0, fb0, fa1, fb1)
        B2S_STEP(kt + 1, fa1, fb1, fa0, fb0)
    }
    if (kt + 1 < nk) {
        B2S_STEP(kt, fa0, fb0, fa1, fb1)
        B2S_MMA16(fa1, fb1)
    } else {
        B2S_MMA16(fa0, fb0)
    }
    asm volatile("s_waitcnt vmcnt(0)" ::: "memory");
#undef B2S_STEP
#undef B2S_MMA16

    gemm_wave_epilogue<4>(g, acc, reinterpret_cast<float*>(smem_raw) + wave * (64 * 64), m0 + wrow, n0 + wcol, lane, z, zo, zi, ksplit, splitk_ws);
}

bf16_t* g_zero_page = nullptr;

__global__ void splitk_reduce_kernel(const float* ws, float* dst, int M, int N, int ldc, int splitk, int conv_dw_cin) {
    const long total = (long)M * N;
    for (long i = ((long)blockIdx.x * blockDim.x + threadIdx.x) * 4; i < total; i += (long)gridDim.x * blockDim.x * 4) {
        float4 acc = *reinterpret_cast<const float4*>(ws + i);
        for (int s = 1; s < splitk; ++s) {
            const float4 v = *reinterpret_cast<const float4*>(ws + (long)s * total + i);
            acc.x += v.x; acc.y += v.y; acc.z += v.z; acc.w += v.w;
        }
        const int m = (int)(i / N), n = (int)(i - (long)m * N);
        const float a4[4] = {acc.x, acc.y, acc.z, acc.w};
        if (conv_dw_cin > 0) {
#pragma unroll
            for (int j = 0; j < 4; ++j) { int nn = n + j, jj = nn / conv_dw_cin; dst[(long)m * ldc + (nn - jj * conv_dw_cin) * 5 + jj] += a4[j]; }
        } else {
            float4* d = reinterpret_cast<float4*>(dst + (long)m * ldc + n);
            float4 c = *d;
            c.x += acc.x; c.y += acc.y; c.z += acc.z; c.w += acc.w;
            *d = c;
        }
    }
}

__global__ __launch_bounds__(256) void splitk_reduce_conv_kernel(const float* __restrict__ ws, float* __restrict__ dst, int M, int N, int ldc, int splitk, int cin) {
    const long total = (long)M * N, pairs = (long)M * cin;
    for (long i = (long)blockIdx.x * blockDim.x + threadIdx.x; i < pairs; i += (long)gridDim.x * blockDim.x) {
        const int m = (int)(i / cin), ci = (int)(i - (long)m * cin);
        float acc[5] = {0.f, 0.f, 0.f, 0.f, 0.f};
        const float* src = ws + (long)m * N + ci;
        for (int s = 0; s < splitk; ++s) {
#pragma unroll
            for (int j = 0; j < 5; ++j) acc[j] += src[(long)s * total + (long)j * cin];
        }
        float* d = dst + (long)m * ldc + (long)ci * 5;
#pragma unroll
        for (int j = 0; j < 5; ++j) d[j] += acc[j];
    }
}

template <bool TA, bool TB, bool GATHER>
int launch_t(const GemmArgs& g_in, hipStream_t stream) {
    GemmArgs g = g_in;
    if (g.splitk > 1) {
        const int nk_all = cdiv(g.K, BK), per = cdiv(nk_all, g.splitk);
        g.splitk = cdiv(nk_all, per);
    }
    constexpr size_t smem = NSTAGE * 2 * (size_t)TILE * sizeof(bf16_t);
    static std::once_flag attr_once;
    static hipError_t attr_err = hipSuccess;
    std::call_once(attr_once, [] {
        attr_err = hipFuncSetAttribute(reinterpret_cast<const void*>(gemm_glds_kernel<TA, TB, GATHER>),
                                       hipFuncAttributeMaxDynamicSharedMemorySize, (int)smem);
    });
    B2S_HIP(attr_err);
    dim3 grid(cdiv(g.N, BN), cdiv(g.M, BM), g.batch * g.splitk);
    float* ws = nullptr;
    if (g.splitk > 1 && g.batch == 1 && g.c_fp32 && g.epi.accumulate && (g.N & 3) == 0 && (g.ldc & 3) == 0 &&
        g.ws && (size_t)g.splitk * g.M * g.N <= g.ws_floats)
        ws = g.ws;
    hipLaunchKernelGGL((gemm_glds_kernel<TA, TB, GATHER>), grid, dim3(256), smem, stream, g, (const bf16_t*)g_zero_page, ws);
    B2S_LAUNCH_CHECK();
    if (ws) B2S_TRY(b2s_splitk_reduce_launch(ws, (float*)g.C, g.M, g.N, g.ldc, g.splitk, g.epi.conv_dw_cin, stream));
    return 0;
}

}

int b2s_splitk_reduce_launch(const float* ws, float* dst, int M, int N, int ldc, int splitk, int conv_dw_cin, hipStream_t stream) {
    if (conv_dw_cin > 0 && N == 5 * conv_dw_cin) {
        const long pairs = (long)M * conv_dw_cin;
        hipLaunchKernelGGL(splitk_reduce_conv_kernel, dim3((int)std::min<long>((pairs + 255) / 256, 2048)), dim3(256), 0, stream, ws, dst, M, N, ldc, splitk,
                           conv_dw_cin);
        B2S_LAUNCH_CHECK();
        return 0;
    }
    const long total4 = (long)M * N / 4;
    int blocks = (int)std::min<long>((total4 + 255) / 256, 2048);
    hipLaunchKernelGGL(splitk_reduce_kernel, dim3(blocks), dim3(256), 0, stream, ws, dst, M, N, ldc, splitk, conv_dw_cin);
    B2S_LAUNCH_CHECK();
    return 0;
// ... 28 lines not shown
```

few-shot-transformer-tts_amd/csrc/gemm_glds256.hip:

```cpp
#include <algorithm>
#include <vector>
#include <cstdlib>
#include <mutex>
#include <atomic>
#include "gemm.h"
#include "gemm_epi.h"

#ifndef B2S_DMA_AUX
#define B2S_DMA_AUX 0
#endif

#ifndef B2S_GROUP_M
#define B2S_GROUP_M 4
#endif
#ifndef B2S_NPROD
#define B2S_NPROD 4
#endif

namespace t256 {

constexpr int NPROD = B2S_NPROD, GROUP_M = B2S_GROUP_M;
constexpr int nprod_of(int gather, int mw = 4) { return gather == 1 ? 0 : NPROD * mw / 4; }
constexpr int nthreads_of(int gather, int mw = 4) { return 64 * (2 * mw + nprod_of(gather, mw)); }
template <int N> __device__ __forceinline__ void wait_vm() { asm volatile("s_waitcnt vmcnt(%0)" ::"n"(N) : "memory"); }
// ... 247 lines not shown
        }
    }
    const unsigned lds_base = (unsigned)(uintptr_t)(lptr_t)smem_raw;
    auto frag_issue = [&](bf16x8_t& dst, bool trans, unsigned addr) {
        if (!trans) {
            asm volatile("ds_read_b128 %0, %1" : "=v"(dst) : "v"(addr) : "memory");
        } else {
            bf16x4_t lo, hi;
            asm volatile("ds_read_b64_tr_b16 %0, %2\n\tds_read_b64_tr_b16 %1, %2 offset:1024"
                         : "=&v"(lo), "=&v"(hi) : "v"(addr) : "memory");
            dst[0] = lo[0]; dst[1] = lo[1]; dst[2] = lo[2]; dst[3] = lo[3];
            dst[4] = hi[0]; dst[5] = hi[1]; dst[6] = hi[2]; dst[7] = hi[3];
        }
    };

    f32x4_t acc[4][NB];
#pragma unroll
    for (int a = 0; a < 4; ++a)
#pragma unroll
        for (int b = 0; b < NB; ++b) acc[a][b] = (f32x4_t){0.f, 0.f, 0.f, 0.f};

#define B2S_MMA16(CA, CB)                                                                                         \
    _Pragma("unroll") for (int a = 0; a < 4; ++a) _Pragma("unroll") for (int b = 0; b < NB; ++b)                  \
        acc[a][b] = __builtin_amdgcn_mfma_f32_16x16x32_bf16(CA[a], CB[b], acc[a][b], 0, 0, 0);
#define B2S_READ8(FA, FB, SLOT, H)                                                                                \
    {                                                                                                              \
        const unsigned sb_ = lds_base + (unsigned)((SLOT) * STG);                                          \
        _Pragma("unroll") for (int t = 0; t < 4; ++t) {                                                            \
            frag_issue(FA[t], TA, sb_ + offA[H][t]);                                                               \
            if (t < NB) frag_issue(FB[t], TB, sb_ + offB[H][t]);                                                   \
        }                                                                                                          \
    }

    if (NP && wave >= NC) {
#pragma unroll
        for (int p = 0; p < NSTAGE; ++p)
            if (p < nk) issue(kt0 + p, p);
        if (nk >= 3) wait_vm<2 * IPW>(); else if (nk == 2) wait_vm<IPW>(); else wait_vm<0>();
        __builtin_amdgcn_s_barrier();
        int slot = 0;
        for (int kt = 0; kt < nk; ++kt) {
            if (kt + 2 < nk) wait_vm<IPW>(); else wait_vm<0>();
            __builtin_amdgcn_s_barrier();
            if (kt + NSTAGE < nk) issue(kt0 + kt + NSTAGE, slot);
            slot = slot + 1 == NSTAGE ? 0 : slot + 1;
        }
        return;
    }

    if (!NP) {
#pragma unroll
        for (int p = 0; p < NSTAGE; ++p) issue(kt0 + p, p);
    }
    bf16x8_t fa0[4], fb0[4], fa1[4], fb1[4];
    if (!NP) { if (six) asm volatile("s_waitcnt vmcnt(12)" ::: "memory"); else asm volatile("s_waitcnt vmcnt(8)" ::: "memory"); }
    __builtin_amdgcn_s_barrier();
    B2S_READ8(fa0, fb0, 0, 0)
    asm volatile("s_waitcnt lgkmcnt(0)" ::: "memory");
    __builtin_amdgcn_sched_barrier(0);

    int slot = 0;
    for (int kt = 0; kt < nk; ++kt) {
        const int nslot = slot + 1 == NSTAGE ? 0 : slot + 1;
        B2S_READ8(fa1, fb1, slot, 1)
        __builtin_amdgcn_sched_barrier(0);
        B2S_MMA16(fa0, fb0)
        __builtin_amdgcn_sched_barrier(0);
        asm volatile("s_waitcnt lgkmcnt(0)" ::: "memory");
        if (!NP) { if (six) asm volatile("s_waitcnt vmcnt(6)" ::: "memory"); else asm volatile("s_waitcnt vmcnt(4)" ::: "memory"); }
        __builtin_amdgcn_s_barrier();
        B2S_READ8(fa0, fb0, nslot, 0)
        __builtin_amdgcn_sched_barrier(0);
        B2S_MMA16(fa1, fb1)
        if (!NP) issue(kt0 + kt + NSTAGE, slot);
        __builtin_amdgcn_sched_barrier(0);
        asm volatile("s_waitcnt lgkmcnt(0)" ::: "memory");
        __builtin_amdgcn_sched_barrier(0);
        slot = nslot;
    }
    if (!NP) asm volatile("s_waitcnt vmcnt(0)" ::: "memory");
#undef B2S_READ8
#undef B2S_MMA16

    gemm_wave_epilogue<NB>(g, acc, reinterpret_cast<float*>(smem_raw) + wave * (64 * 64), m0 + wrow, n0 + wcol, lane, z, zo, zi, ksplit, splitk_ws);
}

template <bool TA, bool TB, int GATHER, int NB, int MW = 4>
__global__ __launch_bounds__(nthreads_of(GATHER, MW), 1) void gemm_glds256_kernel(GemmArgs g, const bf16_t* zero, float* splitk_ws, int tiles_m, int tiles_n) {
    const int wg = xcd_tile_id(blockIdx.x, gridDim.x);
    const int per_z = tiles_n * tiles_m;
    const int bz = wg / per_z, rem = wg - bz * per_z;
    int by, bx;
    if (GROUP_M > 0 && tiles_n >= 16) {
        const int gsz = GROUP_M * tiles_n, grp = rem / gsz, in = rem - grp * gsz;
        const int rows = min(GROUP_M, tiles_m - grp * GROUP_M);
        bx = in / rows; by = grp * GROUP_M + (in - bx * rows);
    } else { by = rem / tiles_n; bx = rem - by * tiles_n; }
    gemm256_body<TA, TB, GATHER, NB, MW>(g, zero, splitk_ws, bx, by, bz);
}

template <int NB, bool SEG = false>
__global__ __launch_bounds__(nthreads_of(false), 1) void gemm_glds256_grouped_kernel(b2s_gemm_group grp, const bf16_t* zero) {
    const int i = blockIdx.x, xcd = i & 7;
    int p = 0, local;
    if (grp.order == 1) {
        const int T = grp.tile0[grp.n];
        int start = 0;
        for (int x = 0; x < xcd; ++x) start += (T - x + 7) >> 3;
        const int g = start + (i >> 3);
        while (p + 1 < grp.n && g >= grp.tile0[p + 1]) ++p;
        local = g - grp.tile0[p];
    } else {
        while (p + 1 < grp.n && i >= grp.tile0[p + 1]) ++p;
        const int s0 = grp.tile0[p], cnt = grp.tile0[p + 1] - s0;
        int before = 0;
        for (int x = 0; x < xcd; ++x) {
            const int first = s0 + ((x - s0) & 7);
            before += first < s0 + cnt ? (s0 + cnt - 1 - first) / 8 + 1 : 0;
        }
        local = before + (i - (s0 + ((xcd - s0) & 7))) / 8;
    }
    const int tiles_tap = (grp.p[p].N + NB * 32 - 1) / (NB * 32);
    const int tiles_n = SEG ? 5 * tiles_tap : tiles_tap, tiles_m = (grp.p[p].M + BM - 1) / BM;
    const int sk = grp.p[p].splitk, t = local / sk, bz = local - t * sk;
    int by, bx;
    if (grp.order == 1 && tiles_n > 8) { bx = t / tiles_m; by = t - bx * tiles_m; }
    else { by = t / tiles_n; bx = t - by * tiles_n; }
    if constexpr (SEG) {
        GemmArgs g = grp.p[p];
        const int j = bx / tiles_tap;
        g.C = reinterpret_cast<float*>(g.C) + j;
        const ConvSeg sg = {grp.seg_len, grp.seg_n, grp.seg_T, j - 2};
        gemm256_body<true, true, 0, NB, 4, true>(g, zero, nullptr, bx - j * tiles_tap, by, 0, sg);
        return;
    }
    gemm256_body<true, true, 0, NB>(grp.p[p], zero, nullptr, bx, by, bz);
}

constexpr int PST_STG = NSTAGE * STAGE_BYTES, PST_TQ = PST_STG + 8 * 1024, PST_LDS = PST_TQ + 64;
constexpr int PST_END = 0x7fffffff;

template <int NB, int MODE>
__device__ __forceinline__ void epi_small(const EpiFast& e, const DropCfg dcfg, f32x4_t (&acc)[4][NB], unsigned stg, int mb, int nb, int lane) {
    typedef uint32_t u32x4 __attribute__((ext_vector_type(4)));
    typedef uint32_t u32x2 __attribute__((ext_vector_type(2)));
    constexpr int CH = NB * 2, TASKS = 8 * CH;
    const int li = lane & 15, lg = lane >> 4;
    const int trow = lane / CH, tch = lane - trow * CH;
    const bool tvalid = lane < TASKS;
    u32x4 qa[MODE == 2 ? 8 : 1];
    if (MODE == 2) {
        const bf16_t* aux = reinterpret_cast<const bf16_t*>(e.relu_aux);
#pragma unroll
        for (int ps = 0; ps < 8; ++ps) {
            const int m = min(mb + ps * 8 + min(trow, 7), e.M - 1);
            qa[ps] = *reinterpret_cast<const u32x4*>(aux + (long)m * e.ld_aux + nb + min(tch, CH - 1) * 8);
        }
    }
    bf16_t* Ct = reinterpret_cast<bf16_t*>(e.C);
    const unsigned wa0 = stg + (unsigned)((li & 7) * 128 + ((((lg >> 1) ^ (li & 7)) << 4) | ((lg & 1) << 3)));
    const unsigned ra = stg + (unsigned)(trow * 128 + ((tch ^ (trow & 7)) << 4));
    constexpr uint32_t HC = 0x9E3779B1u;
    const uint32_t x00 = ((uint32_t)(mb + li) * (uint32_t)e.N + (uint32_t)(nb + lg * 4)) * HC + dcfg.key;
    const uint32_t nc = (uint32_t)e.N * HC;
#pragma unroll
    for (int a = 0; a < 4; ++a) {
        u32x2 pk[NB];
// ... 161 lines not shown
#pragma unroll
    for (int t = 0; t < 4; ++t) {
        const int r = wrow + t * 16 + li;
        offA[0][t] = (unsigned)(r * 128 + ((lg ^ swz_n(r)) << 4)); offA[1][t] = offA[0][t] ^ 64u;
        if (TB) {
            const int k = lg * 8 + (li >> 2), col = wcol + t * 16 + (li & 3) * 4, sw = ((li >> 2) | ((lg & 1) << 2)) << 1;
            const unsigned o = (unsigned)A_B + 2u * (k * 128 + (((col >> 3) ^ sw) << 3) + (col & 7));
            offB[0][t] = o; offB[1][t] = o + UNIT;
        } else {
            const int rb = wcol + t * 16 + li;
            offB[0][t] = (unsigned)(A_B + rb * 128 + ((lg ^ swz_n(rb)) << 4)); offB[1][t] = offB[0][t] ^ 64u;
        }
    }
    auto frag_issue = [&](bf16x8_t& dst, bool trans, unsigned addr) {
        if (!trans) {
            asm volatile("ds_read_b128 %0, %1" : "=v"(dst) : "v"(addr) : "memory");
        } else {
            bf16x4_t lo, hi;
            asm volatile("ds_read_b64_tr_b16 %0, %2\n\tds_read_b64_tr_b16 %1, %2 offset:1024"
                         : "=&v"(lo), "=&v"(hi) : "v"(addr) : "memory");
            dst[0] = lo[0]; dst[1] = lo[1]; dst[2] = lo[2]; dst[3] = lo[3];
            dst[4] = hi[0]; dst[5] = hi[1]; dst[6] = hi[2]; dst[7] = hi[3];
        }
    };
#define B2S_MMA16(CA, CB)                                                                                         \
    _Pragma("unroll") for (int a = 0; a < 4; ++a) _Pragma("unroll") for (int b = 0; b < NB; ++b)                  \
        acc[a][b] = __builtin_amdgcn_mfma_f32_16x16x32_bf16(CB[b], CA[a], acc[a][b], 0, 0, 0);
#define B2S_READ8(FA, FB, SLOT, H)                                                                                \
    {                                                                                                              \
        const unsigned sb_ = lds_base + (unsigned)((SLOT) * STG);                                                  \
        _Pragma("unroll") for (int t = 0; t < 4; ++t) {                                                            \
            frag_issue(FA[t], false, sb_ + offA[H][t]);                                                            \
            if (t < NB) frag_issue(FB[t], TB, sb_ + offB[H][t]);                                                   \
        }                                                                                                          \
    }
    const EpiFast ef = {g.C, g.ldc, g.M, g.N, nullptr, 0, g.epi.relu_aux, g.epi.ld_aux, g.epi.aux_scale, g.epi.drop, g.epi.drop_salt};
    DropCfg dcfg = g.epi.drop;
    if (dcfg.thresh && g.epi.drop_salt) dcfg.key ^= b2s_hash32((uint32_t)(*g.epi.drop_salt) * 2246822519u + 3266489917u);
    const unsigned stg = lds_base + (unsigned)(PST_STG + wave * 1024);
    f32x4_t acc[4][NB];
    bf16x8_t fa0[4], fb0[4], fa1[4], fb1[4];
    __builtin_amdgcn_s_barrier();
    int slot = 0;
    int v = (int)blockIdx.x;
    for (int t = 0; v != PST_END; ++t) {
        int m0, n0; tile_at(v, m0, n0);
#pragma unroll
        for (int a = 0; a < 4; ++a)
#pragma unroll
            for (int b = 0; b < NB; ++b) acc[a][b] = (f32x4_t){0.f, 0.f, 0.f, 0.f};
        B2S_READ8(fa0, fb0, slot, 0)
        asm volatile("s_waitcnt lgkmcnt(0)" ::: "memory");
        __builtin_amdgcn_sched_barrier(0);
        for (int kt = 0; kt < nk; ++kt) {
            const int nslot = slot + 1 == NSTAGE ? 0 : slot + 1;
            B2S_READ8(fa1, fb1, slot, 1)
            __builtin_amdgcn_sched_barrier(0);
            B2S_MMA16(fa0, fb0)
            __builtin_amdgcn_sched_barrier(0);
            asm volatile("s_waitcnt lgkmcnt(0)" ::: "memory");
            __builtin_amdgcn_s_barrier();
            B2S_READ8(fa0, fb0, nslot, 0)
            __builtin_amdgcn_sched_barrier(0);
            B2S_MMA16(fa1, fb1)
            __builtin_amdgcn_sched_barrier(0);
            asm volatile("s_waitcnt lgkmcnt(0)" ::: "memory");
            __builtin_amdgcn_sched_barrier(0);
            slot = nslot;
        }
        __builtin_amdgcn_sched_barrier(0);
        v = queued(t + 1);
        if (mode == 0) epi_small<NB, 0>(ef, dcfg, acc, stg, m0 + wrow, n0 + wcol, lane);
        else if (mode == 1 && !dcfg.thresh) epi_small<NB, 1>(ef, dcfg, acc, stg, m0 + wrow, n0 + wcol, lane);
        else if (mode == 1) epi_small<NB, 3>(ef, dcfg, acc, stg, m0 + wrow, n0 + wcol, lane);
        else epi_small<NB, 2>(ef, dcfg, acc, stg, m0 + wrow, n0 + wcol, lane);
        __builtin_amdgcn_sched_barrier(0);
    }
#undef B2S_READ8
#undef B2S_MMA16
}

inline int persist_mode(const GemmArgs& g) {
    const GemmEpilogue& e = g.epi;
    if (g.c_fp32 || e.residual || e.bias || e.row_len || e.alpha != 1.f || e.kv_k || e.accumulate || e.conv_dw_cin || e.colstat) return -1;
    if ((g.ldc & 7) || (reinterpret_cast<uintptr_t>(g.C) & 15) || g.cs_o || g.cs_i) return -1;
    if (!e.relu && !e.relu_aux && !e.drop.thresh) return 0;
    if (e.relu && !e.relu_aux) return 1;
    if (e.relu_aux && !e.relu && !e.drop.thresh && (e.ld_aux & 7) == 0 && (reinterpret_cast<uintptr_t>(e.relu_aux) & 15) == 0) return 2;
    return -1;
}
#ifdef B2S_LAB
static const int g_persist = getenv("B2S_LAB_GEMM_PERSIST") ? atoi(getenv("B2S_LAB_GEMM_PERSIST")) : 1;
static const int g_persist_min = getenv("B2S_LAB_GEMM_PERSIST_MIN") ? atoi(getenv("B2S_LAB_GEMM_PERSIST_MIN")) : 1;
#else
constexpr int g_persist = 1;
constexpr int g_persist_min = 1;
#endif
int* persist_ticket_set() {
    constexpr int MAXDEV = 16;
    static int* pool[MAXDEV] = {};
    static std::once_flag once[MAXDEV];
    int dev = 0;
    if (hipGetDevice(&dev) != hipSuccess || dev < 0 || dev >= MAXDEV) { (void)hipGetLastError(); return nullptr; }
    std::call_once(once[dev], [dev] {
        void* p = nullptr;
        if (hipMalloc(&p, 1024 * 64) == hipSuccess && hipMemset(p, 0, 1024 * 64) == hipSuccess) pool[dev] = (int*)p;
        else (void)hipGetLastError();
    });
    static std::atomic<unsigned> next{0};
    return pool[dev] ? pool[dev] + (next.fetch_add(1, std::memory_order_relaxed) & 1023u) * 16 : nullptr;
}
template <bool TB, int NB>
int launch256_persist(const GemmArgs& g, int mode, hipStream_t stream) {
    constexpr size_t smem = PST_LDS;
    static std::once_flag attr_once;
    static hipError_t attr_err = hipSuccess;
    std::call_once(attr_once, [] {
        attr_err = hipFuncSetAttribute(reinterpret_cast<const void*>(gemm_glds256_persist_kernel<TB, NB>), hipFuncAttributeMaxDynamicSharedMemorySize, (int)smem);
    });
    B2S_HIP(attr_err);
    const int tiles_m = cdiv(g.M, BM), tiles_n = g.N / (NB * 32);
    int* tickets = (g_persist == 2 || tiles_m * tiles_n <= 256) ? nullptr : persist_ticket_set();
    const int grid = std::min(256, tiles_m * tiles_n);
    hipLaunchKernelGGL((gemm_glds256_persist_kernel<TB, NB>), dim3(grid), dim3(nthreads_of(0, 4)), smem, stream, g, tiles_m, tiles_n, mode, tickets);
    B2S_LAUNCH_CHECK();
    return 0;
}
template <bool TA, bool TB, int GATHER, int NB>
int try_persist(const GemmArgs& g, hipStream_t stream) {
    if (TA || GATHER != 0 || !g_persist) return -1;
    const long tiles = (long)cdiv(g.M, BM) * cdiv(g.N, NB * 32);
    if (tiles < g_persist_min || (tiles < 256 && (tiles & 7)) || tiles >= (1 << 24) || g.batch != 1 || g.splitk != 1 || g.K < 6 * BK || g.K % BK != 0 || g.N % (NB * 32) != 0) return -1;
    if ((long)g.A.R * g.A.ld >= (1L << 30) || (long)g.B.R * g.B.ld >= (1L << 30) || g.A.g_cin || g.B.g_cin) return -1;
    if (TB && !(g.B.C >= 8 && (g.B.C & 7) == 0)) return -1;
    const int mode = persist_mode(g);
    if (mode < 0) return -1;
    return launch256_persist<TB, NB>(g, mode, stream);
}

template <bool TA, bool TB, int GATHER, int NB, int MW = 4>
int launch256_nb(const GemmArgs& g_in, const bf16_t* zero, hipStream_t stream) {
    GemmArgs g = g_in;
    if (g.splitk > 1) {
        const int nk_all = cdiv(g.K, BK), per = cdiv(nk_all, g.splitk);
        g.splitk = cdiv(nk_all, per);
    }
    constexpr size_t smem = (size_t)NSTAGE * (MW * 64 * BK * 2 + B_BYTES);
    static std::once_flag attr_once;
    static hipError_t attr_err = hipSuccess;
    std::call_once(attr_once, [] {
        attr_err = hipFuncSetAttribute(reinterpret_cast<const void*>(gemm_glds256_kernel<TA, TB, GATHER, NB, MW>),
                                       hipFuncAttributeMaxDynamicSharedMemorySize, (int)smem);
    });
    B2S_HIP(attr_err);
    const int tiles_m = cdiv(g.M, MW * 64), tiles_n = cdiv(g.N, NB * 32);
    dim3 grid(tiles_m * tiles_n * g.batch * g.splitk);
    float* ws = nullptr;
    if (g.splitk > 1 && g.batch == 1 && g.c_fp32 && g.epi.accumulate && (g.N & 3) == 0 && (g.ldc & 3) == 0 &&
        g.ws && (size_t)g.splitk * g.M * g.N <= g.ws_floats)
        ws = g.ws;
    hipLaunchKernelGGL((gemm_glds256_kernel<TA, TB, GATHER, NB, MW>), grid, dim3(nthreads_of(GATHER, MW)), smem, stream, g, zero, ws, tiles_m, tiles_n);
    B2S_LAUNCH_CHECK();
    if (ws) B2S_TRY(b2s_splitk_reduce_launch(ws, (float*)g.C, g.M, g.N, g.ldc, g.splitk, g.epi.conv_dw_cin, stream));
    return 0;
}

std::atomic<int> g_tile_policy{0};
inline int pick_nb(const GemmArgs& g, bool allow64 = false) {
    static const int env_force = getenv("B2S_GEMM256_NB") ? atoi(getenv("B2S_GEMM256_NB")) : 0;
    const int force = env_force ? env_force : g_tile_policy.load(std::memory_order_relaxed);
    if (force == 3 || force == 4) return force;
    const long per = (long)cdiv(g.M, BM) * g.batch * std::max(1, g.splitk);
    const long r128 = (per * cdiv(g.N, 128) + 255) / 256 * 128, r96 = (per * cdiv(g.N, 96) + 255) / 256 * 101;
    if (allow64) {
        const long r64 = (per * cdiv(g.N, 64) + 255) / 256 * 72;
        if (r64 < std::min(r96, r128)) return 2;
    }
    return r96 < r128 ? 3 : 4;
}
template <bool TA, bool TB, int GATHER>
int launch256_t(const GemmArgs& g, const bf16_t* zero, hipStream_t stream) {
    if (!TA && GATHER == 0) {
#ifdef B2S_LAB
        static const int small_tiles = getenv("B2S_LAB_SMALL_TILES") ? atoi(getenv("B2S_LAB_SMALL_TILES")) : 128;
#else
        constexpr int small_tiles = 128;
#endif
        const int nb = pick_nb(g);
        const long t256n = (long)cdiv(g.M, BM) * cdiv(g.N, nb * 32) * g.batch * std::max(1, g.splitk);
        if (t256n <= small_tiles && g.M > 128) {
            constexpr bool ta = false;
            return nb == 3 ? launch256_nb<ta, TB, 0, 3, 2>(g, zero, stream)
                           : launch256_nb<ta, TB, 0, 4, 2>(g, zero, stream);
        }
    }
#ifdef B2S_LAB
    static const bool lab_no64 = getenv("B2S_LAB_NO_NB2") != nullptr;
#else
    constexpr bool lab_no64 = false;
#endif
    const int nb = pick_nb(g, GATHER == 2 && !TB && !lab_no64);
    if constexpr (GATHER == 2 && !TB) {
        if (nb == 2) return launch256_nb<TA, TB, GATHER, 2>(g, zero, stream);
    }
    const int rc = nb == 3 ? try_persist<TA, TB, GATHER, 3>(g, stream) : try_persist<TA, TB, GATHER, 4>(g, stream);
    if (rc >= 0) return rc;
    return nb == 3 ? launch256_nb<TA, TB, GATHER, 3>(g, zero, stream)
                   : launch256_nb<TA, TB, GATHER, 4>(g, zero, stream);
}

}

int b2s_gemm_glds256_grouped_launch(const GemmArgs* probs, int n, const bf16_t* zero, hipStream_t stream) {
    B2S_CHECK(n >= 1 && n <= B2S_MAX_GROUP, "grouped GEMM: %d problems (max %d)", n, B2S_MAX_GROUP);
    b2s_gemm_group grp;
    grp.n = n;
    grp.order = 1;
    int order[B2S_MAX_GROUP];
    auto makespan = [&](bool deep_first) {
        for (int i = 0; i < n; ++i) order[i] = i;
        std::stable_sort(order, order + n, [&](int a, int b) { return deep_first ? probs[a].K > probs[b].K : probs[a].K < probs[b].K; });
        std::vector<long> cu(256, 0);
        auto cmp = [](long a, long b) { return a > b; };
        long end = 0;
        for (int k = 0; k < n; ++k) {
            const GemmArgs& g = probs[order[k]];
            const int t = cdiv(g.M, t256::BM) * cdiv(g.N, 128);
            for (int j = 0; j < t; ++j) {
                std::pop_heap(cu.begin(), cu.end(), cmp);
                cu.back() += g.K + 1024;
                end = std::max(end, cu.back());
                std::push_heap(cu.begin(), cu.end(), cmp);
            }
        }
        return end;
    };
    const long deep = makespan(true), shallow = makespan(false);
    if (deep <= shallow) makespan(true);
    int tiles = 0;
    for (int k = 0; k < n; ++k) {
        const GemmArgs& g = probs[order[k]];
        B2S_CHECK(g.batch == 1 && g.c_fp32 && g.A.g_cin == 0 && g.B.g_cin == 0, "grouped GEMM: problem %d is not a plain fp32 dW", order[k]);
        grp.p[k] = g; grp.p[k].splitk = 1;
        grp.tile0[k] = tiles;
        tiles += cdiv(g.M, t256::BM) * cdiv(g.N, 128);
    }
    grp.tile0[n] = tiles;
    grp.seg_len = nullptr; grp.seg_n = 0; grp.seg_T = 0;
    constexpr size_t smem = (size_t)t256::NSTAGE * t256::STAGE_BYTES;
    static std::once_flag attr_once;
    static hipError_t attr_err = hipSuccess;
    std::call_once(attr_once, [] {
        attr_err = hipFuncSetAttribute(reinterpret_cast<const void*>(t256::gemm_glds256_grouped_kernel<4>),
                                       hipFuncAttributeMaxDynamicSharedMemorySize, (int)smem);
    });
    B2S_HIP(attr_err);
    hipLaunchKernelGGL((t256::gemm_glds256_grouped_kernel<4>), dim3(tiles), dim3(t256::nthreads_of(false)), smem, stream, grp, zero);
    B2S_LAUNCH_CHECK();
    return 0;
}

int b2s_gemm_glds256_conv_dw_launch(const GemmArgs* probs, int n, const int* len, int B, int T, const bf16_t* zero, hipStream_t stream) {
    B2S_CHECK(n >= 1 && n <= B2S_MAX_GROUP && B > 0 && T > 0 && (long)B * T < (1L << 30), "conv dW: %d layers (max %d), B = %d, T = %d", n, B2S_MAX_GROUP, B, T);
    b2s_gemm_group grp;
    grp.n = n; grp.order = 1;
    grp.seg_len = len; grp.seg_n = B; grp.seg_T = T;
    int tiles = 0;
    for (int k = 0; k < n; ++k) {
        GemmArgs g = probs[k];
        B2S_CHECK(g.batch == 1 && g.c_fp32 && g.A.p && g.B.p && g.C && g.A.g_cin == 0 && g.B.g_cin == 0, "conv dW: layer %d is not a plain fp32 dW", k);
        B2S_CHECK(g.M > 0 && g.N > 0 && g.M % 8 == 0 && g.N % 8 == 0 && g.A.ld % 8 == 0 && g.B.ld % 8 == 0 && g.A.ld >= g.M && g.B.ld >= g.N && g.ldc >= 5 * g.N,
                  "conv dW: layer %d: cout = %d, cin = %d and the leading dimensions (%d, %d) must be multiples of 8, ldc = %d >= 5 cin", k, g.M, g.N,
                  g.A.ld, g.B.ld, g.ldc);
        B2S_CHECK(((uintptr_t)g.A.p % 16 == 0) && ((uintptr_t)g.B.p % 16 == 0), "conv dW: operands must be 16-byte aligned");
        B2S_CHECK(!g.epi.bias && !g.epi.relu && !g.epi.relu_aux && !g.epi.residual && !g.epi.drop.thresh && !g.epi.row_len && !g.epi.colstat && !g.epi.kv_k,
                  "conv dW: linear epilogue only");
        g.A.R = g.B.R = g.K = B * T; g.A.C = g.M; g.B.C = g.N;
        g.splitk = 1; g.ws = nullptr; g.ws_floats = 0; g.cs_o = g.cs_i = 0; g.A.bs_o = g.A.bs_i = g.B.bs_o = g.B.bs_i = 0;
        g.epi.conv_dw_cin = g.N;
        grp.p[k] = g;
        grp.tile0[k] = tiles;
        tiles += cdiv(g.M, t256::BM) * 5 * cdiv(g.N, 128);
    }
    grp.tile0[n] = tiles;
    constexpr size_t smem = (size_t)t256::NSTAGE * t256::STAGE_BYTES;
    static std::once_flag attr_once;
    static hipError_t attr_err = hipSuccess;
    std::call_once(attr_once, [] {
        attr_err = hipFuncSetAttribute(reinterpret_cast<const void*>(t256::gemm_glds256_grouped_kernel<4, true>),
                                       hipFuncAttributeMaxDynamicSharedMemorySize, (int)smem);
    });
    B2S_HIP(attr_err);
    hipLaunchKernelGGL((t256::gemm_glds256_grouped_kernel<4, true>), dim3(tiles), dim3(t256::nthreads_of(false)), smem, stream, grp, zero);
    B2S_LAUNCH_CHECK();
    return 0;
}

extern "C" int b2s_gemm_set_tile_policy(int policy) {
    if (policy != 0 && policy != 3 && policy != 4) return b2s_fail(__FILE__, __LINE__, "tile policy must be 0 (auto), 3 (256x96) or 4 (256x128), got %d", policy);
    t256::g_tile_policy.store(policy, std::memory_order_relaxed);
    return 0;
}

long b2s_gemm_glds256_tiles(const GemmArgs& g) { return (long)cdiv(g.M, t256::BM) * cdiv(g.N, 128) * g.batch * std::max(1, g.splitk); }

int b2s_gemm_glds256_launch(const GemmArgs& g, bool ta, bool tb, const bf16_t* zero, hipStream_t stream) {
    const bool gather = g.A.g_cin > 0 || g.B.g_cin > 0;
    if (gather) {
        if (!ta && !tb) {
            const bool aligned = g.A.g_cin > 0 && g.B.g_cin == 0 && g.A.g_cin % t256::BK == 0 && g.K % t256::BK == 0 && g.splitk == 1 &&
                                 (long)g.A.R * g.A.ld < (1L << 29) && (long)g.B.R * g.B.ld < (1L << 30) && g.A.g_T > 0;
            if (aligned) return t256::launch256_t<false, false, 2>(g, zero, stream);
            return t256::launch256_t<false, false, 1>(g, zero, stream);
        }
        if (ta && tb) return t256::launch256_t<true, true, 1>(g, zero, stream);
        return b2s_fail(__FILE__, __LINE__, "conv gather is supported for the NT and TN forms only");
    }
    if (!ta && !tb) return t256::launch256_t<false, false, 0>(g, zero, stream);
    if (!ta && tb) return t256::launch256_t<false, true, 0>(g, zero, stream);
    if (ta && !tb) return t256::launch256_t<true, false, 0>(g, zero, stream);
    return t256::launch256_t<true, true, 0>(g, zero, stream);
}
```

few-shot-transformer-tts_amd/csrc/rowops.h:

```cpp
#pragma once
#include "b2s_common.h"

int ro_embed_prep_fwd(const long* ids, const int* lens, const float* embed, const float* pe, const float* pe_scale,
                      float* x, int B, int S, int D, DropCfg drop, hipStream_t st);
int ro_embed_prep_bwd(const float* dx, const long* ids, const int* lens, const float* pe, float* d_embed,
                      float* d_pe_scale, int B, int S, int D, DropCfg drop, hipStream_t st, int dx_bf16 = 0);

int ro_layernorm_fwd(int dtype, const float* x, const float* gamma, const float* beta, void* y, int ldy, float* y32,
                     int ldy32, float* mean, float* rstd, int M, int D, float eps, const int* row_len,
                     int rows_per_batch, hipStream_t st);
int ro_layernorm_bwd(int dtype, const void* dy, int dy_fp32, int lddy, const float* x, const float* gamma,
                     const float* mean, const float* rstd, float* dx, int accumulate, float* dgamma, float* dbeta,
                     int M, int D, const int* row_len, int rows_per_batch, hipStream_t st, float* ws = nullptr,
                     void* dy2 = nullptr, DropCfg drop2 = DropCfg{0, 0, 1.f}, int* defer_nblk = nullptr, int dx_bf16 = 0);
constexpr int RO_LN_WS_ROWS = 768;
struct LnReduceJob { const float* ws; int nblk, D; float* dgamma; float* dbeta; };
constexpr int RO_LN_BATCH = 8;
struct LnReduceBatch { int n; LnReduceJob j[RO_LN_BATCH]; };
int ro_ln_param_reduce_batch(const LnReduceBatch& b, hipStream_t st);

int ro_softmax_fwd(int dtype, const float* S, void* P, void* Pd, int B, int H, int Lq, int Lk, int ldp, float scale,
                   int mask_mode, const int* klen, const float* bias, long bias_sb, long bias_sq, DropCfg drop,
                   hipStream_t st);
int ro_softmax_bwd(int dtype, const void* P, const float* dPraw, void* dS, int B, int H, int Lq, int Lk, int ldp,
                   float scale, DropCfg drop, hipStream_t st);
int ro_align_transpose(int dtype, const void* P, float* align, int Z, int Lq, int Lk, int ldp, hipStream_t st);

int ro_cast_drop(int dtype, const float* in, int ldin, void* out, int ldo, int M, int N, DropCfg drop, hipStream_t st);
int ro_cast(int dtype, const float* in, void* out, long n, hipStream_t st);
int ro_cast_back(int dtype, const void* in, float* out, long n, hipStream_t st);

int ro_shift_pe_fwd(const float* a, const int* lens, const float* pe, const float* pe_scale, float* x, int B, int T,
                    int D, DropCfg drop, hipStream_t st, const int* off = nullptr, int rows = 0);
int ro_shift_pe_bwd(int dtype, const float* dx, const int* lens, const float* pe, void* da, float* d_pe_scale, int B,
                    int T, int D, DropCfg drop, hipStream_t st, int dx_bf16 = 0, const int* off = nullptr, int rows = 0);
int ro_set_rowoff(const int* off_host, int n, int* dst, hipStream_t st);
int ro_rows_gather(int out_dtype, const float* in, void* out, const int* off, int B, int T, int C, hipStream_t st, const float* in2 = nullptr, float* out2 = nullptr, int C2 = 0);
int ro_heads_scatter(int dtype, const void* x, int ldx, const float* w, const float* bias, const float* mel_in, float* mel_out, float* stop_out,
                     const int* off, int B, int T, int C, int D, hipStream_t st);

int ro_spk_embed_fwd(const long* spk_ids, const float* table, const float* W, const float* b, float* e_raw,
                     float* h_pre, float* mem32, void* memT, int dtype, int ldm, int col0, int B, int S, int E,
                     hipStream_t st);
int ro_lang_embed_fwd(const float* vecs, int L, const float* Wl, const float* W, const float* b, float* e_raw,
                      float* h_pre, float* mem32, void* memT, int dtype, int ldm, int col0, int B, int S, int E,
                      hipStream_t st);
int ro_spk_embed_bwd(const float* dmem, int ldm, int col0, const long* spk_ids, const float* e_raw, const float* h_pre,
                     const float* W, float* d_table, float* dW, float* db, float* dh_scratch, int B, int S, int E, hipStream_t st);
int ro_lang_embed_bwd(const float* dmem, int ldm, int col0, const float* vecs, int L, const float* e_raw,
                      const float* h_pre, const float* Wl, const float* W, float* dWl, float* dW, float* db, float* dh_scratch,
                      int B, int S, int E, hipStream_t st);

int ro_rowdot_fwd(int dtype, const void* x, int ldx, const float* w, const float* b, float* out, int M, int D,
                  const int* row_len, int rows_per_batch, hipStream_t st);
int ro_colsum(int dtype, const void* X, int x_fp32, int ldx, const float* wgt, float* out, int accumulate, int M,
              int C, hipStream_t st);

int ro_bn_stats(const float* y, int M, int C, float* mean, float* rstd, float eps, float* running_mean,
                float* running_var, long* num_batches_tracked, float momentum, float* scratch, hipStream_t st);
int ro_bn_apply_train(int dtype, const float* y, const float* sums, float* mean, float* rstd, float eps, float* running_mean, float* running_var,
                      long* num_batches_tracked, float momentum, const float* gamma, const float* beta, int use_tanh, void* outT, float* out32,
                      const float* add32, int M, int C, DropCfg drop, hipStream_t st);
int ro_bn_eval_stats(const float* running_mean, const float* running_var, float* mean, float* rstd, float eps, int C,
                     hipStream_t st);
int ro_bn_apply(int dtype, const float* y, const float* mean, const float* rstd, const float* gamma,
                const float* beta, int use_tanh, void* outT, float* out32, const float* add32, int M, int C,
                DropCfg drop, hipStream_t st);
int ro_bn_bwd(int dtype, const void* dout, int dout_fp32, const float* y, const float* mean, const float* rstd,
              const float* gamma, const float* beta, int use_tanh, float* dgamma, float* dbeta, void* dyT, int M,
              int C, DropCfg drop, hipStream_t st);

int ro_loss_fwd(const float* bef, const float* aft, const float* stop, const float* tgt, const int* lens,
                const float* l2, float* out, float* aft_losses, int B, int T, int C, float pos_weight, float* scratch,
                hipStream_t st, bool scratch_zeroed = false);
int ro_loss_bwd(const float* bef, const float* aft, const float* stop, const float* tgt, const int* lens,
                const float* gscale, float* d_bef, float* d_aft, float* d_stop, int B, int T, int C, float pos_weight,
                hipStream_t st);

struct MtChunk {
    float* a; float* b; float* c; float* d; bf16_t* s; int n; int pad;
    bf16_t* s2; int cin, cout; long off;
};
int ro_mt_sumsq(const MtChunk* chunks, int nchunks, float* out, float scale, hipStream_t st);
int ro_mt_param_wire(const MtChunk* chunks, int nchunks, float* wire, const float* gbase, bool scatter, hipStream_t st);
int ro_mt_cast(const MtChunk* chunks, int nchunks, hipStream_t st);
int ro_mt_zero(const MtChunk* chunks, int nchunks, hipStream_t st);
int ro_mt_axpy(const MtChunk* chunks, int nchunks, float alpha, const float* gscale, hipStream_t st);
struct AdamHyper { float lr, bc1, sbc2; };
int ro_mt_adam(const MtChunk* chunks, int nchunks, AdamHyper hp, float beta1, float beta2, float eps, float l2,
               float grad_scale, float* sumsq_part, hipStream_t st, const void* wire = nullptr, const float* gbase = nullptr,
               int max_wg = 0);
int ro_sum_scaled(const float* part, int n, float scale, float* out, hipStream_t st, float* zero = nullptr, int nzero = 0);

int ro_conv_w_relayout(int dtype, const float* w, void* wf, void* wb, int Cout, int Cin, hipStream_t st);
int ro_add(const float* a, const float* b, float* out, long n, hipStream_t st);
int ro_add3(const float* a, const float* b, const float* c, float* out, long n, hipStream_t st);
```

few-shot-transformer-tts_amd/csrc/rowops.hip:

```cpp
#include <algorithm>
#include <cstdlib>
#include "rowops.h"

namespace {

#define RO_DISPATCH(dtype, CALL) do { if (dtype) { typedef bf16_t TY; CALL; } else { typedef float TY; CALL; } } while (0)

__device__ inline float4 ld4(const float* p) { return *reinterpret_cast<const float4*>(p); }
__device__ inline void st4(float* p, float4 v) { *reinterpret_cast<float4*>(p) = v; }
__device__ inline float4 ld4(const bf16_t* p) {
    uint2 u = *reinterpret_cast<const uint2*>(p);
    return make_float4(bf2f(u.x & 0xffff), bf2f(u.x >> 16), bf2f(u.y & 0xffff), bf2f(u.y >> 16));
}
__device__ inline void st4(bf16_t* p, float4 v) {
    uint2 u;
    u.x = f2bf2(v.x, v.y);
    u.y = f2bf2(v.z, v.w);
    *reinterpret_cast<uint2*>(p) = u;
}
__device__ inline float4 drop4(float4 v, const DropCfg& d, uint32_t idx) {
    if (!d.thresh) return v;
    v.x = b2s_keep(d, idx) ? v.x * d.scale : 0.f;
    v.y = b2s_keep(d, idx + 1) ? v.y * d.scale : 0.f;
    v.z = b2s_keep(d, idx + 2) ? v.z * d.scale : 0.f;
// ... 601 lines not shown
}

__global__ __launch_bounds__(256) void k_bn_colred(const float* y, int M, int C, const float* mu_sum, float* out) {
    __shared__ float sh[4][64];
    const int cx = threadIdx.x & 63, ry = threadIdx.x >> 6;
    const int c = blockIdx.x * 64 + cx;
    float acc = 0.f;
    if (c < C) {
        const float mu = mu_sum ? mu_sum[c] / M : 0.f;
        for (int m = blockIdx.y * 4 + ry; m < M; m += gridDim.y * 4) {
            float v = y[(long)m * C + c];
            if (mu_sum) { v -= mu; v *= v; }
            acc += v;
        }
    }
    sh[ry][cx] = acc;
    __syncthreads();
    if (ry == 0 && c < C) atomicAdd(out + c, sh[0][cx] + sh[1][cx] + sh[2][cx] + sh[3][cx]);
}
__global__ void k_bn_finalize(const float* scratch, int M, int C, float* mean, float* rstd, float eps, float* rm,
                              float* rv, long* nbt, float mom) {
    const int c = blockIdx.x * blockDim.x + threadIdx.x;
    if (c < C) {
        float mu = scratch[c] / M, var = scratch[C + c] / M;
        mean[c] = mu; rstd[c] = 1.f / sqrtf(var + eps);
        if (rm) {
            rm[c] = (1.f - mom) * rm[c] + mom * mu;
            rv[c] = (1.f - mom) * rv[c] + mom * var * ((float)M / (float)(M - 1));
        }
    }
    if (c == 0 && nbt) *nbt += 1;
}
__global__ void k_bn_eval_stats(const float* rm, const float* rv, float* mean, float* rstd, float eps, int C) {
    const int c = blockIdx.x * blockDim.x + threadIdx.x;
    if (c < C) { mean[c] = rm[c]; rstd[c] = 1.f / sqrtf(rv[c] + eps); }
}
template <typename TD>
__device__ inline float bn_dz(const TD* dout, const float* y, long off, int c, const float* mean, const float* rstd,
                              const float* gamma, const float* beta, int use_tanh, const DropCfg& drop, float* xhat) {
    float d = TT<TD>::ld(dout + off);
    if (drop.thresh) d = b2s_keep(drop, (uint32_t)off) ? d * drop.scale : 0.f;
    float xh = (y[off] - mean[c]) * rstd[c];
    *xhat = xh;
    if (use_tanh) { float a = tanhf(gamma[c] * xh + beta[c]); d *= (1.f - a * a); }
    return d;
}
template <typename TD>
__global__ __launch_bounds__(256) void k_bn_bwd_red(const TD* dout, const float* y, const float* mean,
                                                    const float* rstd, const float* gamma, const float* beta,
                                                    int use_tanh, float* dgamma, float* dbeta, int M, int C,
                                                    DropCfg drop) {
    __shared__ float sh[2][4][64];
    const int cx = threadIdx.x & 63, ry = threadIdx.x >> 6;
    const int c = blockIdx.x * 64 + cx;
    float a1 = 0.f, a2 = 0.f;
    if (c < C)
        for (int m = blockIdx.y * 4 + ry; m < M; m += gridDim.y * 4) {
            float xh;
            float dz = bn_dz<TD>(dout, y, (long)m * C + c, c, mean, rstd, gamma, beta, use_tanh, drop, &xh);
            a1 += dz; a2 += dz * xh;
        }
    sh[0][ry][cx] = a1; sh[1][ry][cx] = a2;
    __syncthreads();
    if (ry == 0 && c < C) {
        atomicAdd(dbeta + c, sh[0][0][cx] + sh[0][1][cx] + sh[0][2][cx] + sh[0][3][cx]);
        atomicAdd(dgamma + c, sh[1][0][cx] + sh[1][1][cx] + sh[1][2][cx] + sh[1][3][cx]);
    }
}
template <typename TD, typename T>
__global__ void k_bn_bwd_apply(const TD* dout, const float* y, const float* mean, const float* rstd,
                               const float* gamma, const float* beta, int use_tanh, const float* dgamma,
                               const float* dbeta, T* dy, int M, int C, DropCfg drop) {
    const long total = (long)M * C;
    const float invM = 1.f / M;
    for (long i = (long)blockIdx.x * blockDim.x + threadIdx.x; i < total; i += (long)gridDim.x * blockDim.x) {
        int c = (int)(i % C);
        float xh;
        float dz = bn_dz<TD>(dout, y, i, c, mean, rstd, gamma, beta, use_tanh, drop, &xh);
        TT<T>::st(dy + i, gamma[c] * rstd[c] * (dz - dbeta[c] * invM - xh * dgamma[c] * invM));
    }
}

constexpr int BN_RU = 8;
__device__ __forceinline__ float fast_tanh(float x) { return 1.f - 2.f / (__expf(2.f * x) + 1.f); }
struct BnStat {
    const float* sums;
    float *mean, *rstd;
    float *rm, *rv; long* nbt;
    float eps, mom;
};
template <typename T>
__global__ __launch_bounds__(256) void k_bn_apply_v(const float* __restrict__ y, BnStat bs, const float* __restrict__ gamma, const float* __restrict__ beta,
                                                    int use_tanh, T* __restrict__ outT, float* __restrict__ out32, const float* __restrict__ add32, int M,
                                                    int C, DropCfg drop) {
    const int cq = blockIdx.x * 64 + (threadIdx.x & 63), ry = threadIdx.x >> 6;
    const int c = min(cq * 4, C - 4);
    const bool own = cq * 4 < C;
    float4 mu, rs;
    if (bs.sums) {
        const float4 s1 = ld4(bs.sums + c), s2 = ld4(bs.sums + C + c);
        const float im = 1.f / M;
        mu = make_float4(s1.x * im, s1.y * im, s1.z * im, s1.w * im);
        const float4 var = make_float4(fmaxf(s2.x * im - mu.x * mu.x, 0.f), fmaxf(s2.y * im - mu.y * mu.y, 0.f), fmaxf(s2.z * im - mu.z * mu.z, 0.f),
                                       fmaxf(s2.w * im - mu.w * mu.w, 0.f));
        rs = make_float4(1.f / sqrtf(var.x + bs.eps), 1.f / sqrtf(var.y + bs.eps), 1.f / sqrtf(var.z + bs.eps), 1.f / sqrtf(var.w + bs.eps));
        if (blockIdx.y == 0 && ry == 0 && own) {
            st4(bs.mean + c, mu); st4(bs.rstd + c, rs);
            if (bs.rm) {
                const float unb = (float)M / (float)(M - 1), a = 1.f - bs.mom, b = bs.mom;
                const float4 m0 = ld4(bs.rm + c), v0 = ld4(bs.rv + c);
                st4(bs.rm + c, make_float4(a * m0.x + b * mu.x, a * m0.y + b * mu.y, a * m0.z + b * mu.z, a * m0.w + b * mu.w));
                st4(bs.rv + c, make_float4(a * v0.x + b * var.x * unb, a * v0.y + b * var.y * unb, a * v0.z + b * var.z * unb, a * v0.w + b * var.w * unb));
            }
            if (bs.nbt && cq == 0) *bs.nbt += 1;
        }
    } else { mu = ld4(bs.mean + c); rs = ld4(bs.rstd + c); }
    const float4 g = ld4(gamma + c), be = ld4(beta + c);
    const int m0 = (blockIdx.y * 4 + ry) * BN_RU;
    float4 v[BN_RU], ad[BN_RU];
#pragma unroll
    for (int j = 0; j < BN_RU; ++j) {
        const long o = (long)min(m0 + j, M - 1) * C + c;
        v[j] = ld4(y + o);
        if (add32) ad[j] = ld4(add32 + o);
    }
#pragma unroll
    for (int j = 0; j < BN_RU; ++j) {
        const int m = m0 + j;
        float4 o;
        o.x = (v[j].x - mu.x) * rs.x * g.x + be.x; o.y = (v[j].y - mu.y) * rs.y * g.y + be.y;
        o.z = (v[j].z - mu.z) * rs.z * g.z + be.z; o.w = (v[j].w - mu.w) * rs.w * g.w + be.w;
        if (use_tanh) { o.x = fast_tanh(o.x); o.y = fast_tanh(o.y); o.z = fast_tanh(o.z); o.w = fast_tanh(o.w); }
        o = drop4(o, drop, (uint32_t)((long)m * C + c));
        if (m < M && own) {
            if (outT) st4(outT + (long)m * C + c, o);
            if (out32) {
                if (add32) { o.x += ad[j].x; o.y += ad[j].y; o.z += ad[j].z; o.w += ad[j].w; }
                st4(out32 + (long)m * C + c, o);
            }
        }
    }
}
template <typename TD>
__device__ __forceinline__ float4 bn_dz4(float4 d, float4 yv, float4 mu, float4 rs, float4 g, float4 be, int use_tanh, const DropCfg& drop, uint32_t off,
                                         float4* xh) {
    d = drop4(d, drop, off);
    *xh = make_float4((yv.x - mu.x) * rs.x, (yv.y - mu.y) * rs.y, (yv.z - mu.z) * rs.z, (yv.w - mu.w) * rs.w);
    if (use_tanh) {
        const float a0 = fast_tanh(g.x * xh->x + be.x), a1 = fast_tanh(g.y * xh->y + be.y), a2 = fast_tanh(g.z * xh->z + be.z), a3 = fast_tanh(g.w * xh->w + be.w);
        d.x *= 1.f - a0 * a0; d.y *= 1.f - a1 * a1; d.z *= 1.f - a2 * a2; d.w *= 1.f - a3 * a3;
    }
    return d;
}
template <typename TD, typename T, bool APPLY>
__global__ __launch_bounds__(256) void k_bn_bwd_v(const TD* __restrict__ dout, const float* __restrict__ y, const float* __restrict__ mean,
                                                  const float* __restrict__ rstd, const float* __restrict__ gamma, const float* __restrict__ beta,
                                                  int use_tanh, float* dgamma, float* dbeta, T* __restrict__ dy, int M, int C, DropCfg drop) {
    __shared__ float sh[2][4][256];
    const int cx = threadIdx.x & 63, cq = blockIdx.x * 64 + cx, ry = threadIdx.x >> 6;
    const int c = min(cq * 4, C - 4);
    const bool own = cq * 4 < C;
    const float4 mu = ld4(mean + c), rs = ld4(rstd + c), g = ld4(gamma + c), be = ld4(beta + c);
    float4 sg = make_float4(0, 0, 0, 0), sb = make_float4(0, 0, 0, 0);
    if (APPLY) { sg = ld4(dgamma + c); sb = ld4(dbeta + c); }
    const int m0 = (blockIdx.y * 4 + ry) * BN_RU;
    float4 dv[BN_RU], yv[BN_RU];
#pragma unroll
// ... 500 lines not shown
    int th = ((E + 63) / 64) * 64;
    RO_DISPATCH(dtype, hipLaunchKernelGGL((k_embed_net_fwd<TY>), dim3(B), dim3(th), E * sizeof(float), st,
                                          (const long*)nullptr, (const float*)nullptr, vecs, L, Wl, W, b, e_raw, h_pre,
                                          mem32, (TY*)memT, ldm, col0, S, E));
    B2S_LAUNCH_CHECK(); return 0;
}
int ro_spk_embed_bwd(const float* dmem, int ldm, int col0, const long* spk_ids, const float* e_raw, const float* h_pre,
                     const float* W, float* d_table, float* dW, float* db, float* dh_scratch, int B, int S, int E, hipStream_t st) {
    int th = ((E + 63) / 64) * 64;
    float* de = dh_scratch + (long)B * E;
    hipLaunchKernelGGL(k_embed_net_bwd_dh, dim3(B), dim3(E * std::max(1, 1024 / E)), 0, st, dmem, ldm, col0, h_pre, dh_scratch, S, E);
    hipLaunchKernelGGL(k_embed_net_bwd_de, dim3(B), dim3(th), E * sizeof(float), st, (const float*)dh_scratch, spk_ids, W, de, d_table, E);
    hipLaunchKernelGGL(k_embed_net_bwd_w, dim3(E), dim3(th), 0, st, (const float*)dh_scratch, (const float*)de, e_raw,
                       (const float*)nullptr, 0, dW, db, (float*)nullptr, B, E);
    B2S_LAUNCH_CHECK(); return 0;
}
int ro_lang_embed_bwd(const float* dmem, int ldm, int col0, const float* vecs, int L, const float* e_raw,
                      const float* h_pre, const float* Wl, const float* W, float* dWl, float* dW, float* db, float* dh_scratch,
                      int B, int S, int E, hipStream_t st) {
    (void)Wl;
    int th = ((std::max(E, L) + 63) / 64) * 64;
    float* de = dh_scratch + (long)B * E;
    hipLaunchKernelGGL(k_embed_net_bwd_dh, dim3(B), dim3(E * std::max(1, 1024 / E)), 0, st, dmem, ldm, col0, h_pre, dh_scratch, S, E);
    hipLaunchKernelGGL(k_embed_net_bwd_de, dim3(B), dim3(th), E * sizeof(float), st, (const float*)dh_scratch, (const long*)nullptr, W, de,
                       (float*)nullptr, E);
    hipLaunchKernelGGL(k_embed_net_bwd_w, dim3(E), dim3(th), 0, st, (const float*)dh_scratch, (const float*)de, e_raw, vecs, L, dW, db, dWl,
                       B, E);
    B2S_LAUNCH_CHECK(); return 0;
}
int ro_rowdot_fwd(int dtype, const void* x, int ldx, const float* w, const float* b, float* out, int M, int D,
                  const int* row_len, int rows_per_batch, hipStream_t st) {
    B2S_CHECK(D % 4 == 0, "rowdot: D=%d must be a multiple of 4", D);
    RO_DISPATCH(dtype, hipLaunchKernelGGL((k_rowdot<TY>), dim3(cdiv(M, 4)), dim3(256), 0, st, (const TY*)x, ldx, w, b, out,
                                          M, D, row_len, rows_per_batch));
    B2S_LAUNCH_CHECK(); return 0;
}
int ro_colsum(int dtype, const void* X, int x_fp32, int ldx, const float* wgt, float* out, int accumulate, int M,
              int C, hipStream_t st) {
    if (!accumulate) B2S_HIP(hipMemsetAsync(out, 0, sizeof(float) * C, st));
    int gy = cdiv(M, 4 * 16); if (gy > 128) gy = 128; if (gy < 1) gy = 1;
    dim3 grid(cdiv(C, 64), gy);
    if (x_fp32 || !dtype)
        hipLaunchKernelGGL((k_colsum<float>), grid, dim3(256), 0, st, (const float*)X, ldx, wgt, out, M, C);
    else
        hipLaunchKernelGGL((k_colsum<bf16_t>), grid, dim3(256), 0, st, (const bf16_t*)X, ldx, wgt, out, M, C);
    B2S_LAUNCH_CHECK(); return 0;
}
int ro_bn_stats(const float* y, int M, int C, float* mean, float* rstd, float eps, float* running_mean,
                float* running_var, long* num_batches_tracked, float momentum, float* scratch, hipStream_t st) {
    B2S_HIP(hipMemsetAsync(scratch, 0, sizeof(float) * 2 * C, st));
    int gy = cdiv(M, 4 * 16); if (gy > 128) gy = 128; if (gy < 1) gy = 1;
    dim3 grid(cdiv(C, 64), gy);
    hipLaunchKernelGGL(k_bn_colred, grid, dim3(256), 0, st, y, M, C, (const float*)nullptr, scratch);
    hipLaunchKernelGGL(k_bn_colred, grid, dim3(256), 0, st, y, M, C, (const float*)scratch, scratch + C);
    hipLaunchKernelGGL(k_bn_finalize, dim3(cdiv(C, 256)), dim3(256), 0, st, (const float*)scratch, M, C, mean, rstd, eps,
                       running_mean, running_var, num_batches_tracked, momentum);
    B2S_LAUNCH_CHECK(); return 0;
}
int ro_bn_eval_stats(const float* running_mean, const float* running_var, float* mean, float* rstd, float eps, int C,
                     hipStream_t st) {
    hipLaunchKernelGGL(k_bn_eval_stats, dim3(cdiv(C, 256)), dim3(256), 0, st, running_mean, running_var, mean, rstd, eps, C);
    B2S_LAUNCH_CHECK(); return 0;
}
int ro_bn_apply_train(int dtype, const float* y, const float* sums, float* mean, float* rstd, float eps, float* running_mean, float* running_var,
                      long* num_batches_tracked, float momentum, const float* gamma, const float* beta, int use_tanh, void* outT, float* out32,
                      const float* add32, int M, int C, DropCfg drop, hipStream_t st) {
    B2S_CHECK(C % 4 == 0 && M > 1, "bn_apply_train: C=%d must be a multiple of 4, M=%d > 1", C, M);
    BnStat bs = {sums, mean, rstd, running_mean, running_var, num_batches_tracked, eps, momentum};
    dim3 grid(cdiv(C / 4, 64), cdiv(M, 4 * BN_RU));
    RO_DISPATCH(dtype, hipLaunchKernelGGL((k_bn_apply_v<TY>), grid, dim3(256), 0, st, y, bs, gamma, beta, use_tanh, (TY*)outT, out32, add32, M, C, drop));
    B2S_LAUNCH_CHECK(); return 0;
}
int ro_bn_apply(int dtype, const float* y, const float* mean, const float* rstd, const float* gamma,
                const float* beta, int use_tanh, void* outT, float* out32, const float* add32, int M, int C,
                DropCfg drop, hipStream_t st) {
    B2S_CHECK(C % 4 == 0, "bn_apply: C=%d must be a multiple of 4", C);
    BnStat bs = {nullptr, const_cast<float*>(mean), const_cast<float*>(rstd), nullptr, nullptr, nullptr, 0.f, 0.f};
    dim3 grid(cdiv(C / 4, 64), cdiv(M, 4 * BN_RU));
    RO_DISPATCH(dtype, hipLaunchKernelGGL((k_bn_apply_v<TY>), grid, dim3(256), 0, st, y, bs, gamma, beta, use_tanh, (TY*)outT, out32, add32, M, C, drop));
    B2S_LAUNCH_CHECK(); return 0;
}
int ro_bn_bwd(int dtype, const void* dout, int dout_fp32, const float* y, const float* mean, const float* rstd,
              const float* gamma, const float* beta, int use_tanh, float* dgamma, float* dbeta, void* dyT, int M,
              int C, DropCfg drop, hipStream_t st) {
    if (C % 4 == 0) {
        dim3 gv(cdiv(C / 4, 64), cdiv(M, 4 * BN_RU));
#define B2S_BN_BWD(TD, T) do { \
        hipLaunchKernelGGL((k_bn_bwd_v<TD, T, false>), gv, dim3(256), 0, st, (const TD*)dout, y, mean, rstd, gamma, beta, use_tanh, dgamma, dbeta, (T*)dyT, M, C, drop); \
        hipLaunchKernelGGL((k_bn_bwd_v<TD, T, true>), gv, dim3(256), 0, st, (const TD*)dout, y, mean, rstd, gamma, beta, use_tanh, dgamma, dbeta, (T*)dyT, M, C, drop); } while (0)
        if (dout_fp32 || !dtype) { if (dtype) B2S_BN_BWD(float, bf16_t); else B2S_BN_BWD(float, float); }
        else B2S_BN_BWD(bf16_t, bf16_t);
#undef B2S_BN_BWD
        B2S_LAUNCH_CHECK(); return 0;
    }
    int gy = cdiv(M, 4 * 16); if (gy > 128) gy = 128; if (gy < 1) gy = 1;
    dim3 grid(cdiv(C, 64), gy);
    const int g2 = ew_grid((long)M * C);
    if (dout_fp32 || !dtype) {
        hipLaunchKernelGGL((k_bn_bwd_red<float>), grid, dim3(256), 0, st, (const float*)dout, y, mean, rstd, gamma, beta,
                           use_tanh, dgamma, dbeta, M, C, drop);
        RO_DISPATCH(dtype, hipLaunchKernelGGL((k_bn_bwd_apply<float, TY>), dim3(g2), dim3(256), 0, st, (const float*)dout,
                                              y, mean, rstd, gamma, beta, use_tanh, (const float*)dgamma,
                                              (const float*)dbeta, (TY*)dyT, M, C, drop));
    } else {
        hipLaunchKernelGGL((k_bn_bwd_red<bf16_t>), grid, dim3(256), 0, st, (const bf16_t*)dout, y, mean, rstd, gamma,
                           beta, use_tanh, dgamma, dbeta, M, C, drop);
        hipLaunchKernelGGL((k_bn_bwd_apply<bf16_t, bf16_t>), dim3(g2), dim3(256), 0, st, (const bf16_t*)dout, y, mean,
                           rstd, gamma, beta, use_tanh, (const float*)dgamma, (const float*)dbeta, (bf16_t*)dyT, M, C,
                           drop);
    }
    B2S_LAUNCH_CHECK(); return 0;
}
int ro_loss_fwd(const float* bef, const float* aft, const float* stop, const float* tgt, const int* lens,
                const float* l2, float* out, float* aft_losses, int B, int T, int C, float pos_weight, float* scratch,
                hipStream_t st, bool scratch_zeroed) {
    if (!scratch_zeroed) B2S_HIP(hipMemsetAsync(scratch, 0, sizeof(float) * (3 + B), st));
    if (C % 4 == 0)
        hipLaunchKernelGGL(k_loss_partial_v, dim3(std::max(1, std::min(cdiv((long)T * C / 4, 1024), 16)), B), dim3(256), 0, st, bef, aft, stop, tgt, lens,
                           scratch, T, C, pos_weight);
    else
        hipLaunchKernelGGL(k_loss_partial, dim3(std::min(cdiv(T, 4), 32), B), dim3(256), 0, st, bef, aft, stop, tgt, lens, scratch, B,
                           T, C, pos_weight);
    hipLaunchKernelGGL(k_loss_finalize, dim3(1), dim3(64), 0, st, (const float*)scratch, lens, l2, out, aft_losses, B);
    B2S_LAUNCH_CHECK(); return 0;
}
int ro_loss_bwd(const float* bef, const float* aft, const float* stop, const float* tgt, const int* lens,
                const float* gscale, float* d_bef, float* d_aft, float* d_stop, int B, int T, int C, float pos_weight,
                hipStream_t st) {
    hipLaunchKernelGGL(k_loss_bwd, dim3(cdiv((long)B * T, 4)), dim3(256), 0, st, bef, aft, stop, tgt, lens, gscale, d_bef,
                       d_aft, d_stop, B, T, C, pos_weight);
    B2S_LAUNCH_CHECK(); return 0;
}
int ro_mt_sumsq(const MtChunk* chunks, int nchunks, float* out, float scale, hipStream_t st) {
    if (nchunks > 0) hipLaunchKernelGGL(k_mt_sumsq, dim3(nchunks), dim3(256), 0, st, chunks, out, scale);
    B2S_LAUNCH_CHECK(); return 0;
}
int ro_mt_axpy(const MtChunk* chunks, int nchunks, float alpha, const float* gscale, hipStream_t st) {
    if (nchunks > 0) hipLaunchKernelGGL(k_mt_axpy, dim3(nchunks), dim3(256), 0, st, chunks, alpha, gscale);
    B2S_LAUNCH_CHECK(); return 0;
}
int ro_mt_adam(const MtChunk* chunks, int nchunks, AdamHyper hp, float beta1, float beta2, float eps, float l2,
               float grad_scale, float* sumsq_part, hipStream_t st, const void* wire, const float* gbase, int max_wg) {
    constexpr bool v1 = false;
    const int grid = max_wg > 0 ? std::min(max_wg, nchunks) : nchunks;
    if (nchunks > 0 && wire)
        hipLaunchKernelGGL(k_mt_adam2<true>, dim3(grid), dim3(256), 0, st, chunks, nchunks, hp, beta1, beta2, eps, l2, grad_scale, sumsq_part, (const bf16_t*)wire, gbase);
    else if (nchunks > 0 && v1)
        hipLaunchKernelGGL(k_mt_adam, dim3(nchunks), dim3(256), 0, st, chunks, hp, beta1, beta2, eps, l2, grad_scale, sumsq_part);
    else if (nchunks > 0)
        hipLaunchKernelGGL(k_mt_adam2<false>, dim3(grid), dim3(256), 0, st, chunks, nchunks, hp, beta1, beta2, eps, l2, grad_scale, sumsq_part, (const bf16_t*)nullptr,
                           (const float*)nullptr);
    B2S_LAUNCH_CHECK(); return 0;
}
int ro_sum_scaled(const float* part, int n, float scale, float* out, hipStream_t st, float* zero, int nzero) {
    hipLaunchKernelGGL(k_sum_scaled, dim3(1), dim3(1024), 0, st, part, n, scale, out, zero, nzero);
    B2S_LAUNCH_CHECK(); return 0;
}
int ro_conv_w_relayout(int dtype, const float* w, void* wf, void* wb, int Cout, int Cin, hipStream_t st) {
    RO_DISPATCH(dtype, hipLaunchKernelGGL((k_conv_w_relayout<TY>), dim3(ew_grid((long)Cout * Cin * 5)), dim3(256), 0, st, w,
                                          (TY*)wf, (TY*)wb, Cout, Cin));
    B2S_LAUNCH_CHECK(); return 0;
}
int ro_add3(const float* a, const float* b, const float* c, float* out, long n, hipStream_t st) {
    hipLaunchKernelGGL(k_add3, dim3(ew_grid(n)), dim3(256), 0, st, a, b, c, out, n);
    B2S_LAUNCH_CHECK(); return 0;
}
int ro_add(const float* a, const float* b, float* out, long n, hipStream_t st) {
    hipLaunchKernelGGL(k_add, dim3(ew_grid(n)), dim3(256), 0, st, a, b, out, n);
    B2S_LAUNCH_CHECK(); return 0;
}
__global__ __launch_bounds__(256) void k_mt_cast(const MtChunk* __restrict__ ch) {
// ... 70 lines not shown
```

include/b2s_hip.h:

```cpp
#ifndef B2S_HIP_H
#define B2S_HIP_H
#include <stddef.h>
#include <stdint.h>

#ifdef __cplusplus
extern "C" {
#endif

#define B2S_DTYPE_FP32 0
#define B2S_DTYPE_BF16 1

const char* b2s_last_error(void);
int b2s_version(void);

typedef struct b2s_config {
    int32_t num_mels, vocab_size, embed_size, encoder_hidden, decoder_hidden;
    int32_t n_encoder_layer, n_decoder_layer, n_attention_head;
    int32_t prenet_hidden, postnet_hidden, n_postnet_layer;
    int32_t multi_speaker, max_num_speaker, speaker_embedding_size;
    int32_t multi_lingual, max_num_language, language_embedding_size;
    float transformer_dropout_rate, decoder_dropout_rate;
    float reg_weight;
    int32_t compute_dtype;
    float guided_attention_weight, guided_attention_sigma;
// ... 10 lines not shown
int b2s_model_bind(b2s_model* m, void* const* data_host, void* const* grad_host, int n);
int b2s_model_sync_weights(b2s_model* m, void* stream, int shadows_fresh);

size_t b2s_encoder_ws_bytes(const b2s_model* m, int B, int S);
int b2s_encoder_forward(b2s_model* m, const int64_t* inputs, const int32_t* input_lengths, const int64_t* spk_ids,
                        const float* language_vecs, int B, int S, int train, uint64_t seed, void* ws, size_t ws_bytes,
                        float* memory_out, void* stream, b2s_ctx** ctx_out);
int b2s_encoder_backward(b2s_model* m, b2s_ctx* ctx, const float* d_memory, void* stream);

int b2s_decoder_compact_rows(b2s_model* m, const int32_t* target_lengths_host, int B);

size_t b2s_decoder_ws_bytes(const b2s_model* m, int B, int S, int T);
#define B2S_DEC_PADDED_UNOBSERVED 2
int b2s_decoder_forward(b2s_model* m, const float* memory, const int32_t* input_lengths, const float* targets,
                        const int32_t* target_lengths, int B, int S, int T, int train, uint64_t seed, void* ws,
                        size_t ws_bytes, float* mels_out, float* stop_out, void* memory_ready, void* stream, b2s_ctx** ctx_out);
#define B2S_DEC_BWD_NO_DMEMORY 1
#define B2S_DEC_BWD_DEFER_JOIN 2
#define B2S_DEC_BWD_FLUSH_TAIL 4
int b2s_decoder_backward(b2s_model* m, b2s_ctx* ctx, const float* d_mels, const float* d_stop, const float* d_guided,
                         int flags, float* d_memory_out, void* dmem_done, void* stream);
int b2s_decoder_guided_loss(b2s_model* m, b2s_ctx* ctx, float* out, float* add_to, void* stream);
int b2s_decoder_alignment(b2s_model* m, b2s_ctx* ctx, int which, int layer, float* out, void* stream);

size_t b2s_postnet_ws_bytes(const b2s_model* m, int B, int T);
int b2s_postnet_forward(b2s_model* m, const float* inputs, const int32_t* lengths, const float* add, int B, int T,
                        int train, uint64_t seed, void* ws, size_t ws_bytes, float* out, void* stream,
                        b2s_ctx** ctx_out);
#define B2S_POST_BWD_DEFER_JOIN 1
int b2s_postnet_backward(b2s_model* m, b2s_ctx* ctx, const float* d_out, float* d_inputs_out, int flags, void* stream);

void b2s_ctx_free(b2s_ctx* ctx);

int b2s_model_set_stage_hook(b2s_model* m, void (*hook)(int stage, void* user), void* user, void* stream);
void* b2s_model_second_stream(b2s_model* m);
int b2s_model_set_side_stream(b2s_model* m, void* stream);
int b2s_model_backward_abort(b2s_model* m, void* stream);
int b2s_gemm_set_tile_policy(int policy);

int b2s_loss_forward(b2s_model* m, const float* mel_bef, const float* mel_aft, const float* stop_logits,
                     const float* mel_targets, const int32_t* target_lengths, int B, int T, float* losses_out,
                     float* aft_losses_out, float* scratch, void* stream);
int b2s_loss_backward(b2s_model* m, const float* mel_bef, const float* mel_aft, const float* stop_logits,
                      const float* mel_targets, const int32_t* target_lengths, int B, int T, const float* w,
                      float* d_bef, float* d_aft, float* d_stop, void* stream);
int b2s_l2_backward(b2s_model* m, const float* grad_scale, void* stream);

typedef struct b2s_decode_state b2s_decode_state;
size_t b2s_decode_ws_bytes(const b2s_model* m, int B, int S, int max_frames, int keep_self_alignments);
int b2s_decode_begin(b2s_model* m, const float* memory, const int32_t* input_lengths, int B, int S, int max_frames, int train,
                     uint64_t seed, int keep_self_alignments, void* ws, size_t ws_bytes, void* stream, b2s_decode_state** out);
int b2s_decode_run(b2s_model* m, b2s_decode_state* s, int n_steps, int use_graph, void* stream);
int b2s_decode_status(b2s_decode_state* s, int* frames_host, int* all_finished_host, void* stream);
int b2s_decode_fetch(b2s_model* m, b2s_decode_state* s, int n_frames, float* mels_out, int32_t* lengths_out, void* stream);
int b2s_decode_alignment(b2s_model* m, b2s_decode_state* s, int which, int layer, int n_frames, float* align_out, void* stream);
void b2s_decode_end(b2s_decode_state* s);

int b2s_adam_bind(b2s_model* m, void* const* exp_avg_host, void* const* exp_avg_sq_host, int n);
int b2s_adam_step(b2s_model* m, float lr, int step, float beta1, float beta2, float eps, float l2, float grad_scale,
                  void* stream);
int b2s_adam_set_grad_wire(b2s_model* m, const void* wire_bf16, const float* grad_base);
#define B2S_ADAM_ENCODER 1
#define B2S_ADAM_DECODER 2
#define B2S_ADAM_POSTNET 4
int b2s_adam_step_groups(b2s_model* m, float lr, int step, float beta1, float beta2, float eps, float l2, float grad_scale,
                         int groups, int behind_mark, void* stream);
int b2s_model_mark_grads_ready(b2s_model* m);
int b2s_adam_shard(b2s_model* m, const float* grad_base, const int64_t* lo, const int64_t* hi, int n);
int b2s_param_wire(b2s_model* m, float* wire, int direction, void* stream);
#define B2S_ZERO_GRADS_OVERWRITE_DW 1
int b2s_zero_grads(b2s_model* m, void* stream, int flags);
int b2s_model_set_grad_slot_padding(b2s_model* m, int bytes);

typedef struct b2s_gemm_desc {
    int32_t dtype, trans_a, trans_b, M, N, K, lda, ldb, ldc, c_fp32;
    int32_t batch, batch_inner;
    int64_t a_bs_o, a_bs_i, b_bs_o, b_bs_i, c_bs_o, c_bs_i;
    float alpha;
    int32_t relu, accumulate;
    float drop_p;
    uint64_t seed;
    int32_t conv_cin_a, conv_T, conv_dw_cin;
    int32_t rows_per_batch;
} b2s_gemm_desc;
int b2s_gemm(const b2s_gemm_desc* d, const void* A, const void* B, void* C, const float* bias, const float* residual,
             const int32_t* row_len, const int32_t* conv_len, void* stream);
int b2s_gemm_splitk(const b2s_gemm_desc* d, int splitk, const void* A, const void* B, float* C, float* ws, size_t ws_floats,
                    void* stream);
int b2s_layernorm_forward(int dtype, const float* x, const float* gamma, const float* beta, void* y, float* mean,
                          float* rstd, int M, int D, float eps, void* stream);
int b2s_layernorm_backward(int dtype, const void* dy, const float* x, const float* gamma, const float* mean,
                           const float* rstd, float* dx, float* dgamma, float* dbeta, int M, int D, void* stream);
size_t b2s_attention_ws_bytes(int dtype, int B, int H, int Lq, int Lk);
int b2s_attention_forward(int dtype, const void* q, int ldq, const void* k, int ldk, const void* v, int ldv, void* ctx,
                          int ldc, int B, int H, int Lq, int Lk, int dh, int mask_mode, const int32_t* klen,
                          const float* bias, int64_t bias_sb, int64_t bias_sq, float drop_p, uint64_t seed, void* ws,
                          void* P_out, void* Pd_out, void* stream);
int b2s_attention_backward(int dtype, const void* dctx, int ldc, const void* q, int ldq, const void* k, int ldk,
                           const void* v, int ldv, const void* P, const void* Pd, void* dq, int lddq, void* dk,
                           int lddk, void* dv, int lddv, int B, int H, int Lq, int Lk, int dh, float drop_p,
                           uint64_t seed, void* ws, void* stream);
int b2s_flash_attention_forward(int dtype, const void* q, int ldq, const void* k, int ldk, const void* v, int ldv, void* ctx,
                                int ldc, int B, int H, int Lq, int Lk, int dh, int mask_mode, const int32_t* klen,
                                float drop_p, uint64_t seed, float* lse_out, void* stream);
int b2s_flash_attention_backward(int dtype, const void* dctx, const void* ctx, int ldc, const void* q, int ldq,
                                 const void* k, int ldk, const void* v, int ldv, const float* lse, float* dsum_scratch,
                                 void* dq, int lddq, void* dk, int lddk, void* dv, int lddv, int B, int H, int Lq,
                                 int Lk, int dh, int mask_mode, const int32_t* klen, float drop_p, uint64_t seed,
                                 void* stream);
int b2s_flash_attention_align(int dtype, const void* q, int ldq, const void* k, int ldk, const float* lse, int B, int H,
                              int Lq, int Lk, int dh, int mask_mode, const int32_t* klen, float* align_out, void* stream);
int b2s_align_from_probs(int dtype, const void* P, float* align, int B, int H, int Lq, int Lk, void* stream);
int b2s_add3(const float* a, const float* b, const float* c, float* out, int64_t n, void* stream);
int b2s_cast(int dtype, const float* in, void* out, int64_t n, void* stream);
int b2s_cast_back(int dtype, const void* in, float* out, int64_t n, void* stream);
int b2s_dropout_mask(float p, uint64_t seed, uint32_t op_id, uint8_t* out, int64_t n, void* stream);
int b2s_dropout_mask_attn(float p, uint64_t seed, uint32_t op_id, uint8_t* out, int64_t rows, int Lk, void* stream);
int b2s_dropout_site(const char* site, int layer, int decode, uint32_t* op_id_out, int* kind_out, int* salt_out);

void b2s_prof_enable(int on);
int b2s_prof_collect(double* out, int n_variants);

int b2s_encf_attention_forward(const void* hN, const void* Wqkv, const void* Wo, const int32_t* klen, int B, int S, float drop_p, uint64_t seed,
                               uint32_t op_id, void* qkv, void* ctx, float* lse, void* slabs, int slab_bf16, void* stream);
int b2s_encf_attention_backward(const void* dY, const void* qkv, const void* ctx, const float* lse, const void* WoT, const void* WqkvT,
                                const int32_t* klen, int B, int S, float drop_p, uint64_t seed, uint32_t op_id, void* dqkv, void* slabs, int slab_bf16,
                                void* stream);
int b2s_encf_ffn_sublayer(int backward, const void* X, const void* Wa, const void* Wb, void* f_io, void* dz, int B, int S, float drop_p, uint64_t seed,
                          uint32_t op_id, void* slabs, int slab_bf16, void* stream);
int b2s_encf_reduce_layernorm_forward(const float* x_in, const void* slabs, int ns, int slab_bf16, float drop_p, uint64_t seed, uint32_t op_id,
                                      const float* gamma, const float* beta, float* x_out, void* h, float* h32, int ldh32, float* mean, float* rstd,
                                      int M, void* stream);
int b2s_encf_reduce_layernorm_backward(const void* slabs, int ns, int slab_bf16, const float* x_in, const float* gamma, const float* mean,
                                       const float* rstd, float* dx, float* dgamma, float* dbeta, float* ws, void* dy2, float drop_p, uint64_t seed,
                                       uint32_t op_id, int M, void* stream);
int b2s_transpose_bf16(const void* src, void* dst, int R, int C, void* stream);

#ifdef __cplusplus
}
#endif
#endif
```

Measured before the change: 1.239 million mel-frames/s.

## Fuse postnet BatchNorm backward reductions into the conv dX GEMM epilogue

New measurement: 1.237 million mel-frames/s. About the same (-0.2%).

```diff
diff --git a/few-shot-transformer-tts_amd/b2s_hip/lib.py b/few-shot-transformer-tts_amd/b2s_hip/lib.py
--- a/few-shot-transformer-tts_amd/b2s_hip/lib.py
+++ b/few-shot-transformer-tts_amd/b2s_hip/lib.py
@@ -33,7 +33,8 @@
                [(n, C.c_int64) for n in ("a_bs_o", "a_bs_i", "b_bs_o", "b_bs_i", "c_bs_o", "c_bs_i")] + \
                [("alpha", C.c_float), ("relu", C.c_int32), ("accumulate", C.c_int32), ("drop_p", C.c_float),
                 ("seed", C.c_uint64), ("conv_cin_a", C.c_int32), ("conv_T", C.c_int32), ("conv_dw_cin", C.c_int32),
-                ("rows_per_batch", C.c_int32)]
+                ("rows_per_batch", C.c_int32), ("bn_mode", C.c_int32), ("bn_tanh", C.c_int32), ("bn_drop_p", C.c_float), ("bn_op_id", C.c_uint32)] + \
+               [(n, C.c_void_p) for n in ("bn_y", "bn_mean", "bn_rstd", "bn_gamma", "bn_beta", "bn_dgamma", "bn_dbeta", "bn_dy")]
 
 
 P = C.c_void_p
diff --git a/few-shot-transformer-tts_amd/b2s_hip/ops.py b/few-shot-transformer-tts_amd/b2s_hip/ops.py
--- a/few-shot-transformer-tts_amd/b2s_hip/ops.py
+++ b/few-shot-transformer-tts_amd/b2s_hip/ops.py
@@ -29,7 +29,7 @@
 def gemm(dtype, A, B, M, N, K, trans_a=False, trans_b=False, out=None, c_fp32=True, lda=None, ldb=None, ldc=None,
          bias=None, relu=False, residual=None, accumulate=False, alpha=1.0, batch=1, batch_inner=1,
          a_bs=(0, 0), b_bs=(0, 0), c_bs=(0, 0), row_len=None, rows_per_batch=1, conv_cin_a=0, conv_T=0, conv_len=None,
-         conv_dw_cin=0, drop_p=0.0, seed=0):
+         conv_dw_cin=0, drop_p=0.0, seed=0, bn=None):
     d = L.GemmDesc()
     d.dtype, d.trans_a, d.trans_b, d.M, d.N, d.K = dtype, int(trans_a), int(trans_b), M, N, K
     d.lda = lda if lda is not None else (M if trans_a else K)
@@ -42,6 +42,10 @@
     d.c_bs_o, d.c_bs_i = c_bs
     d.alpha, d.relu, d.accumulate, d.drop_p, d.seed = alpha, int(relu), int(accumulate), drop_p, seed
     d.conv_cin_a, d.conv_T, d.conv_dw_cin, d.rows_per_batch = conv_cin_a, conv_T, conv_dw_cin, rows_per_batch
+    if bn:
+        d.bn_mode, d.bn_tanh, d.bn_drop_p, d.bn_op_id = int(bn["mode"]), int(bn.get("tanh", 1)), float(bn.get("drop_p", 0.0)), int(bn.get("op_id", 0))
+        for k in ("y", "mean", "rstd", "gamma", "beta", "dgamma", "dbeta", "dy"):
+            setattr(d, "bn_" + k, L.ptr(bn.get(k)))
     if out is None:
         shape = (batch, M, d.ldc) if batch > 1 else (M, d.ldc)
         out = torch.empty(shape, dtype=torch.float32 if c_fp32 or not dtype else torch.int16, device=A.device)
diff --git a/few-shot-transformer-tts_amd/csrc/b2s_common.h b/few-shot-transformer-tts_amd/csrc/b2s_common.h
--- a/few-shot-transformer-tts_amd/csrc/b2s_common.h
+++ b/few-shot-transformer-tts_amd/csrc/b2s_common.h
@@ -82,6 +82,8 @@
     return d;
 }
 
+__device__ __forceinline__ float b2s_fast_tanh(float x) { return 1.f - 2.f / (__expf(2.f * x) + 1.f); }
+
 __device__ inline float wave_sum(float v) {
 #pragma unroll
     for (int o = 32; o > 0; o >>= 1) v += __shfl_xor(v, o, 64);
diff --git a/few-shot-transformer-tts_amd/csrc/capi_ops.hip b/few-shot-transformer-tts_amd/csrc/capi_ops.hip
--- a/few-shot-transformer-tts_amd/csrc/capi_ops.hip
+++ b/few-shot-transformer-tts_amd/csrc/capi_ops.hip
@@ -47,6 +47,20 @@
         w.C = C; w.c_fp32 = 1; w.ldc = d->ldc; w.epi.accumulate = d->accumulate;
         return b2s_gemm_conv_dw_launch(&w, 1, conv_len, d->K / d->conv_T, d->conv_T, S_(stream));
     }
+    if (d->bn_mode) {
+        B2S_CHECK((d->bn_mode == 1 || d->bn_mode == 2) && d->dtype == 1 && d->conv_cin_a > 0 && !d->c_fp32 && d->ldc == d->N && d->bn_y && d->bn_mean &&
+                  d->bn_rstd && d->bn_gamma && d->bn_beta && d->bn_dgamma && d->bn_dbeta && (d->bn_mode == 1 || d->bn_dy),
+                  "bn_mode: bf16 conv dX with a dense bf16 output, all BatchNorm operands given (bn_mode = 2 needs bn_dy)");
+        const DropCfg bd = make_drop(d->bn_drop_p, d->seed, d->bn_op_id);
+        if (d->bn_mode == 1) {
+            g.epi.bn_y = d->bn_y; g.epi.bn_mean = d->bn_mean; g.epi.bn_rstd = d->bn_rstd; g.epi.bn_gamma = d->bn_gamma; g.epi.bn_beta = d->bn_beta;
+            g.epi.bn_tanh = d->bn_tanh; g.epi.bn_drop = bd; g.epi.bn_dgamma = d->bn_dgamma; g.epi.bn_dbeta = d->bn_dbeta;
+        }
+        B2S_TRY(b2s_gemm_launch(g, d->dtype, d->trans_a != 0, d->trans_b != 0, S_(stream)));
+        if (!d->bn_dy) return 0;
+        return ro_bn_bwd(1, C, 0, d->bn_y, d->bn_mean, d->bn_rstd, d->bn_gamma, d->bn_beta, d->bn_tanh, d->bn_dgamma, d->bn_dbeta, d->bn_dy, d->M, d->N, bd,
+                         S_(stream), d->bn_mode == 1);
+    }
     return b2s_gemm_launch(g, d->dtype, d->trans_a != 0, d->trans_b != 0, S_(stream));
 }
 extern "C" int b2s_gemm_splitk(const b2s_gemm_desc* d, int splitk, const void* A, const void* B, float* C, float* ws, size_t ws_floats,
diff --git a/few-shot-transformer-tts_amd/csrc/engine.hip b/few-shot-transformer-tts_amd/csrc/engine.hip
--- a/few-shot-transformer-tts_amd/csrc/engine.hip
+++ b/few-shot-transformer-tts_amd/csrc/engine.hip
@@ -1844,6 +1844,7 @@
     b2s_ctx tmp; tmp.B = B; tmp.T = T;
     PostScratch ps;
     plan_postnet(m, tmp, a, ps);
+    bool have_sums = false;
     std::vector<GemmArgs> dws, segs;
     for (int i = n - 1; i >= 0; --i) {
         const int cin = i == 0 ? cf.num_mels : cf.postnet_hidden, cout = i == n - 1 ? cf.num_mels : cf.postnet_hidden;
@@ -1852,7 +1853,8 @@
         const void* dout = i == n - 1 ? (const void*)d_out : ps.du[i + 1];
         void* dy = ps.dy[i];
         B2S_TRY(ro_bn_bwd(dt, dout, i == n - 1 ? 1 : 0, c->y[i], c->bn_mean[i], c->bn_rstd[i], m->P(q + "weight"), m->P(q + "bias"),
-                          i < n - 1 ? 1 : 0, m->G(q + "weight"), m->G(q + "bias"), dy, (int)M, cout, d, st));
+                          i < n - 1 ? 1 : 0, m->G(q + "weight"), m->G(q + "bias"), dy, (int)M, cout, d, st, have_sums));
+        have_sums = false;
         if (dt == 1 && cin % 8 == 0 && cout % 8 == 0) {
             GemmArgs g;
             g.A.p = dy; g.A.ld = cout; g.B.p = c->u[i]; g.B.ld = cin;
@@ -1878,6 +1880,14 @@
             g.epi.row_len = c->tgt_len; g.epi.rows_per_batch = T;
             if (i == 0) { g.C = d_inputs_out; g.c_fp32 = 1; } else { g.C = ps.du[i]; g.c_fp32 = 0; }
             g.ldc = cin;
+            if (i > 0 && dt == 1 && cin % 8 == 0) {
+                const std::string p = "postnet.batchnorm_layers." + std::to_string(i - 1) + ".";
+                g.epi.bn_y = c->y[i - 1]; g.epi.bn_mean = c->bn_mean[i - 1]; g.epi.bn_rstd = c->bn_rstd[i - 1];
+                g.epi.bn_gamma = m->P(p + "weight"); g.epi.bn_beta = m->P(p + "bias"); g.epi.bn_tanh = 1;
+                g.epi.bn_drop = make_drop(pd, c->seed, drop_op(DS_POST_CONV, i - 1));
+                g.epi.bn_dgamma = m->G(p + "weight"); g.epi.bn_dbeta = m->G(p + "bias");
+                have_sums = true;
+            }
             B2S_TRY(b2s_gemm_launch(g, dt, false, false, st));
         }
     }
diff --git a/few-shot-transformer-tts_amd/csrc/gemm.h b/few-shot-transformer-tts_amd/csrc/gemm.h
--- a/few-shot-transformer-tts_amd/csrc/gemm.h
+++ b/few-shot-transformer-tts_amd/csrc/gemm.h
@@ -26,6 +26,11 @@
     int conv_dw_cin = 0;
     int accumulate = 0;
     float* colstat = nullptr;
+    const float* bn_y = nullptr;
+    const float *bn_mean = nullptr, *bn_rstd = nullptr, *bn_gamma = nullptr, *bn_beta = nullptr;
+    float *bn_dgamma = nullptr, *bn_dbeta = nullptr;
+    int bn_tanh = 0;
+    DropCfg bn_drop = {0, 0, 1.f};
     void *kv_k = nullptr, *kv_v = nullptr;
     const int* kv_t = nullptr;
     int kv_maxT = 0, kv_D = 0, kv_dh = 0;
diff --git a/few-shot-transformer-tts_amd/csrc/gemm.hip b/few-shot-transformer-tts_amd/csrc/gemm.hip
--- a/few-shot-transformer-tts_amd/csrc/gemm.hip
+++ b/few-shot-transformer-tts_amd/csrc/gemm.hip
@@ -289,6 +289,10 @@
                                                    !g.epi.relu_aux && !g.epi.drop.thresh)),
               "gemm: split-K needs a linear fp32 accumulate epilogue");
     B2S_CHECK(!g.epi.kv_k, "gemm: the cache-append fusion exists in the decode-step kernel only (M <= 64, K %% 32 == 0)");
+    B2S_CHECK(!g.epi.bn_y || (dtype == 1 && !ta && !tb && g.A.g_cin > 0 && !g.c_fp32 && g.N % 8 == 0 && g.batch == 1 && g.splitk == 1 && !g.epi.residual &&
+                              !g.epi.accumulate && !g.epi.conv_dw_cin && !g.epi.bias && !g.epi.relu && !g.epi.relu_aux && !g.epi.drop.thresh &&
+                              g.epi.alpha == 1.f && !g.epi.colstat && g.epi.bn_mean && g.epi.bn_rstd && g.epi.bn_gamma && g.epi.bn_beta && g.epi.bn_dgamma && g.epi.bn_dbeta),
+              "gemm: the BatchNorm backward sums are taken by the bf16 conv gather GEMM (NN form, bf16 output, N %% 8 == 0) with a plain or row-masked store");
     if (!dtype) return launch_fp32(g, ta, tb, stream);
     static const long min_m = getenv("B2S_GEMM256_MIN_M") ? atol(getenv("B2S_GEMM256_MIN_M")) : 129;
     if (g.batch == 1 && g.M >= min_m) {
diff --git a/few-shot-transformer-tts_amd/csrc/gemm_epi.h b/few-shot-transformer-tts_amd/csrc/gemm_epi.h
--- a/few-shot-transformer-tts_amd/csrc/gemm_epi.h
+++ b/few-shot-transformer-tts_amd/csrc/gemm_epi.h
@@ -111,6 +111,37 @@
 }
 
 template <int NB>
+__device__ __forceinline__ void epi_bn_sums(const GemmArgs& g, const float* stg, int mb, int nb, int lane) {
+    const GemmEpilogue& e = g.epi;
+    constexpr int ROWS = NB == 2 ? 32 : 64, RB = 16;
+    const int col = NB == 2 ? (lane & 31) : lane, r_base = NB == 2 ? (lane >> 5) * 32 : 0;
+    const int n = nb + col;
+    const bool act = col < NB * 16 && n < g.N;
+    const int nn = act ? n : 0;
+    const float mu = e.bn_mean[nn], rs = e.bn_rstd[nn], ga = e.bn_gamma[nn], be = e.bn_beta[nn];
+    float s1 = 0.f, s2 = 0.f;
+#pragma unroll 1
+    for (int r0 = 0; r0 < ROWS; r0 += RB) {
+        float yv[RB];
+#pragma unroll
+        for (int j = 0; j < RB; ++j) yv[j] = e.bn_y[(long)min(mb + r_base + r0 + j, g.M - 1) * g.N + nn];
+#pragma unroll
+        for (int j = 0; j < RB; ++j) {
+            const int row = r_base + r0 + j, m = min(mb + row, g.M - 1);
+            bool live = act && mb + row < g.M;
+            if (e.row_len) { const int bb = m / e.rows_per_batch; live = live && (m - bb * e.rows_per_batch) < e.row_len[bb]; }
+            float d = bf2f(f2bf(stg[row * 64 + (col ^ (((row >> 2) & 1) << 4))]));
+            if (e.bn_drop.thresh) d = b2s_keep(e.bn_drop, (uint32_t)((long)m * g.N + nn)) ? d * e.bn_drop.scale : 0.f;
+            const float xh = (yv[j] - mu) * rs;
+            if (e.bn_tanh) { const float a = b2s_fast_tanh(ga * xh + be); d *= 1.f - a * a; }
+            if (live) { s1 += d; s2 += d * xh; }
+        }
+    }
+    if (NB == 2) { s1 += __shfl_xor(s1, 32, 64); s2 += __shfl_xor(s2, 32, 64); }
+    if (act && r_base == 0) { atomicAdd(e.bn_dbeta + n, s1); atomicAdd(e.bn_dgamma + n, s2); }
+}
+
+template <int NB, bool BNS = false>
 __device__ __forceinline__ void gemm_wave_epilogue(GemmArgs g, f32x4_t (&acc)[4][NB], float* stg, int mb, int nb, int lane, int z, int zo, int zi,
                                           int ksplit, float* splitk_ws) {
     const int li = lane & 15, lg = lane >> 4;
@@ -119,7 +150,7 @@
     {
         const GemmEpilogue& e = g.epi;
         const long cb = zo * g.cs_o + zi * g.cs_i;
-        const bool common = g.splitk == 1 && e.conv_dw_cin == 0 && !e.accumulate && !e.bias && !e.row_len && e.alpha == 1.f && !e.kv_k &&
+        const bool common = g.splitk == 1 && e.conv_dw_cin == 0 && !e.accumulate && !e.bias && !e.row_len && e.alpha == 1.f && !e.kv_k && !e.bn_y &&
                             mb + 64 <= g.M && nb + NB * 16 <= g.N && (g.ldc & 7) == 0 && (cb & 7) == 0 &&
                             (reinterpret_cast<uintptr_t>(g.C) & 15) == 0;
         if (common) {
@@ -291,4 +322,5 @@
         }
     }
     }
+    if (BNS && e.bn_y) epi_bn_sums<NB>(g, stg, mb, nb, lane);
 }
diff --git a/few-shot-transformer-tts_amd/csrc/gemm_glds.hip b/few-shot-transformer-tts_amd/csrc/gemm_glds.hip
--- a/few-shot-transformer-tts_amd/csrc/gemm_glds.hip
+++ b/few-shot-transformer-tts_amd/csrc/gemm_glds.hip
@@ -158,7 +158,7 @@
 #undef B2S_STEP
 #undef B2S_MMA16
 
-    gemm_wave_epilogue<4>(g, acc, reinterpret_cast<float*>(smem_raw) + wave * (64 * 64), m0 + wrow, n0 + wcol, lane, z, zo, zi, ksplit, splitk_ws);
+    gemm_wave_epilogue<4, (GATHER && !TA && !TB)>(g, acc, reinterpret_cast<float*>(smem_raw) + wave * (64 * 64), m0 + wrow, n0 + wcol, lane, z, zo, zi, ksplit, splitk_ws);
 }
 
 bf16_t* g_zero_page = nullptr;
diff --git a/few-shot-transformer-tts_amd/csrc/gemm_glds256.hip b/few-shot-transformer-tts_amd/csrc/gemm_glds256.hip
--- a/few-shot-transformer-tts_amd/csrc/gemm_glds256.hip
+++ b/few-shot-transformer-tts_amd/csrc/gemm_glds256.hip
@@ -353,7 +353,7 @@
 #undef B2S_READ8
 #undef B2S_MMA16
 
-    gemm_wave_epilogue<NB>(g, acc, reinterpret_cast<float*>(smem_raw) + wave * (64 * 64), m0 + wrow, n0 + wcol, lane, z, zo, zi, ksplit, splitk_ws);
+    gemm_wave_epilogue<NB, (GATHER != 0 && !TA && !TB && !SEG)>(g, acc, reinterpret_cast<float*>(smem_raw) + wave * (64 * 64), m0 + wrow, n0 + wcol, lane, z, zo, zi, ksplit, splitk_ws);
 }
 
 template <bool TA, bool TB, int GATHER, int NB, int MW = 4>
@@ -681,7 +681,7 @@
 
 inline int persist_mode(const GemmArgs& g) {
     const GemmEpilogue& e = g.epi;
-    if (g.c_fp32 || e.residual || e.bias || e.row_len || e.alpha != 1.f || e.kv_k || e.accumulate || e.conv_dw_cin || e.colstat) return -1;
+    if (g.c_fp32 || e.residual || e.bias || e.row_len || e.alpha != 1.f || e.kv_k || e.accumulate || e.conv_dw_cin || e.colstat || e.bn_y) return -1;
     if ((g.ldc & 7) || (reinterpret_cast<uintptr_t>(g.C) & 15) || g.cs_o || g.cs_i) return -1;
     if (!e.relu && !e.relu_aux && !e.drop.thresh) return 0;
     if (e.relu && !e.relu_aux) return 1;
@@ -810,6 +810,7 @@
 
 }
 
+static_assert(sizeof(b2s_gemm_group) <= 4096, "the grouped launches pass their problem list by value: HIP kernel arguments end at 4 KB");
 int b2s_gemm_glds256_grouped_launch(const GemmArgs* probs, int n, const bf16_t* zero, hipStream_t stream) {
     B2S_CHECK(n >= 1 && n <= B2S_MAX_GROUP, "grouped GEMM: %d problems (max %d)", n, B2S_MAX_GROUP);
     b2s_gemm_group grp;
@@ -872,7 +873,7 @@
                   "conv dW: layer %d: cout = %d, cin = %d and the leading dimensions (%d, %d) must be multiples of 8, ldc = %d >= 5 cin", k, g.M, g.N,
                   g.A.ld, g.B.ld, g.ldc);
         B2S_CHECK(((uintptr_t)g.A.p % 16 == 0) && ((uintptr_t)g.B.p % 16 == 0), "conv dW: operands must be 16-byte aligned");
-        B2S_CHECK(!g.epi.bias && !g.epi.relu && !g.epi.relu_aux && !g.epi.residual && !g.epi.drop.thresh && !g.epi.row_len && !g.epi.colstat && !g.epi.kv_k,
+        B2S_CHECK(!g.epi.bias && !g.epi.relu && !g.epi.relu_aux && !g.epi.residual && !g.epi.drop.thresh && !g.epi.row_len && !g.epi.colstat && !g.epi.kv_k && !g.epi.bn_y,
                   "conv dW: linear epilogue only");
         g.A.R = g.B.R = g.K = B * T; g.A.C = g.M; g.B.C = g.N;
         g.splitk = 1; g.ws = nullptr; g.ws_floats = 0; g.cs_o = g.cs_i = 0; g.A.bs_o = g.A.bs_i = g.B.bs_o = g.B.bs_i = 0;
diff --git a/few-shot-transformer-tts_amd/csrc/rowops.h b/few-shot-transformer-tts_amd/csrc/rowops.h
--- a/few-shot-transformer-tts_amd/csrc/rowops.h
+++ b/few-shot-transformer-tts_amd/csrc/rowops.h
@@ -68,7 +68,7 @@
                 DropCfg drop, hipStream_t st);
 int ro_bn_bwd(int dtype, const void* dout, int dout_fp32, const float* y, const float* mean, const float* rstd,
               const float* gamma, const float* beta, int use_tanh, float* dgamma, float* dbeta, void* dyT, int M,
-              int C, DropCfg drop, hipStream_t st);
+              int C, DropCfg drop, hipStream_t st, bool have_sums = false);
 
 int ro_loss_fwd(const float* bef, const float* aft, const float* stop, const float* tgt, const int* lens,
                 const float* l2, float* out, float* aft_losses, int B, int T, int C, float pos_weight, float* scratch,
diff --git a/few-shot-transformer-tts_amd/csrc/rowops.hip b/few-shot-transformer-tts_amd/csrc/rowops.hip
--- a/few-shot-transformer-tts_amd/csrc/rowops.hip
+++ b/few-shot-transformer-tts_amd/csrc/rowops.hip
@@ -707,7 +707,7 @@
 }
 
 constexpr int BN_RU = 8;
-__device__ __forceinline__ float fast_tanh(float x) { return 1.f - 2.f / (__expf(2.f * x) + 1.f); }
+__device__ __forceinline__ float fast_tanh(float x) { return b2s_fast_tanh(x); }
 struct BnStat {
     const float* sums;
     float *mean, *rstd;
@@ -1374,11 +1374,12 @@
 }
 int ro_bn_bwd(int dtype, const void* dout, int dout_fp32, const float* y, const float* mean, const float* rstd,
               const float* gamma, const float* beta, int use_tanh, float* dgamma, float* dbeta, void* dyT, int M,
-              int C, DropCfg drop, hipStream_t st) {
+              int C, DropCfg drop, hipStream_t st, bool have_sums) {
+    B2S_CHECK(!have_sums || C % 4 == 0, "bn_bwd: sums taken by a GEMM epilogue imply C %% 8 == 0 (C = %d)", C);
     if (C % 4 == 0) {
         dim3 gv(cdiv(C / 4, 64), cdiv(M, 4 * BN_RU));
 #define B2S_BN_BWD(TD, T) do { \
-        hipLaunchKernelGGL((k_bn_bwd_v<TD, T, false>), gv, dim3(256), 0, st, (const TD*)dout, y, mean, rstd, gamma, beta, use_tanh, dgamma, dbeta, (T*)dyT, M, C, drop); \
+        if (!have_sums) hipLaunchKernelGGL((k_bn_bwd_v<TD, T, false>), gv, dim3(256), 0, st, (const TD*)dout, y, mean, rstd, gamma, beta, use_tanh, dgamma, dbeta, (T*)dyT, M, C, drop); \
         hipLaunchKernelGGL((k_bn_bwd_v<TD, T, true>), gv, dim3(256), 0, st, (const TD*)dout, y, mean, rstd, gamma, beta, use_tanh, dgamma, dbeta, (T*)dyT, M, C, drop); } while (0)
         if (dout_fp32 || !dtype) { if (dtype) B2S_BN_BWD(float, bf16_t); else B2S_BN_BWD(float, float); }
         else B2S_BN_BWD(bf16_t, bf16_t);
diff --git a/include/b2s_hip.h b/include/b2s_hip.h
--- a/include/b2s_hip.h
+++ b/include/b2s_hip.h
@@ -116,6 +116,12 @@
     uint64_t seed;
     int32_t conv_cin_a, conv_T, conv_dw_cin;
     int32_t rows_per_batch;
+    int32_t bn_mode, bn_tanh;
+    float bn_drop_p;
+    uint32_t bn_op_id;
+    const float *bn_y, *bn_mean, *bn_rstd, *bn_gamma, *bn_beta;
+    float *bn_dgamma, *bn_dbeta;
+    void* bn_dy;
 } b2s_gemm_desc;
 int b2s_gemm(const b2s_gemm_desc* d, const void* A, const void* B, void* C, const float* bias, const float* residual,
              const int32_t* row_len, const int32_t* conv_len, void* stream);
```
